# facebookresearch/SONAR

Hardware: NVIDIA B200
Metric: sentences/sec->1024-d (higher is better)
Workload: dtype bf16

## Files before the change

include/sonar_b200.h:

```cpp
#ifndef SONAR_B200_H_
#define SONAR_B200_H_

#include <stddef.h>
#include <stdint.h>

#ifdef __cplusplus
extern "C" {
#endif

#define SB_OK 0
#define SB_ERR_INVALID (-1)
#define SB_ERR_CUDA (-2)
#define SB_ERR_DRIVER (-3)
#define SB_ERR_INPUT (-4)

#define SB_POOL_MAX 1
#define SB_POOL_MEAN 2
#define SB_POOL_LAST 3

#define SB_EPI_BIAS 0
#define SB_EPI_BIAS_RELU 1
#define SB_EPI_BIAS_RESIDUAL 2
#define SB_EPI_BIAS_SILU 5

typedef struct SbEncoder SbEncoder;

typedef struct SbEncoderConfig {
  int32_t model_dim;
  int32_t num_layers;
  int32_t num_heads;
  int32_t ffn_inner_dim;
  int64_t vocab_size;
  int32_t pos_rows;
  int32_t pooling;
  float ln_eps;
  float embed_scale;
  int32_t cta_group;
  int32_t num_sms;
  int32_t ln_fold;
  int32_t epi_groups;
} SbEncoderConfig;

typedef struct SbLayerWeights {
  const void* wqkv;
  const float* bqkv;
  const void* wo;
  const float* bo;
  const void* w1;
  const float* b1;
  const void* w2;
  const float* b2;
  const float* ln1_g;
  const float* ln1_b;
  const float* ln2_g;
  const float* ln2_b;
} SbLayerWeights;

typedef struct SbEncoderWeights {
  const void* embed;
  const float* pos_table;
  const float* final_ln_g;
  const float* final_ln_b;
  const SbLayerWeights* layers;
} SbEncoderWeights;

const char* sb_last_error(void);
int sb_version(void);

int sb_encoder_create(const SbEncoderConfig* cfg, const SbEncoderWeights* w, SbEncoder** out);
void sb_encoder_destroy(SbEncoder* enc);

int sb_encoder_workspace_bytes(const SbEncoder* enc, int32_t max_batch, int64_t max_tokens, size_t* bytes);

int sb_encoder_forward(SbEncoder* enc, const int64_t* ids, int64_t ids_row_stride, const int32_t* seq_lens_host,
                       int32_t batch, int32_t seq_len, float* out, float* encoded, void* workspace,
                       size_t workspace_bytes, void* stream);

int sb_encoder_forward_host(SbEncoder* enc, const int64_t* ids_host, const int32_t* seq_lens_host, int32_t batch,
                            int32_t seq_len, float* out_host, int64_t* ids_staging, float* out_staging,
                            void* workspace, size_t workspace_bytes, void* stream);

int sb_encoder_profile_ffn1(SbEncoder* enc, void* start_event, void* stop_event);

int sb_encoder_check_inputs(SbEncoder* enc, void* workspace, void* stream);


int sb_fold_layernorm(const void* W, const float* bias, const float* gamma, const float* beta, int32_t N, int32_t K,
                      void* Wf, float* colsum, float* bias_f, void* stream);
int sb_gemm_ln_consumer(const void* A, int64_t lda, const void* Wf, int64_t ldw, void* C, int64_t ldc, const float* bias_f,
                        const float* colsum, const float* stats, float eps, int32_t M, int32_t N, int32_t K, int32_t relu,
                        void* stream);
int sb_gemm_residual_stats(const void* A, int64_t lda, const void* W, int64_t ldw, float* x, int64_t ldx, const float* bias,
                           void* h_out, int64_t ldh, float* stats_out, int32_t M, int32_t N, int32_t K, void* stream);

int sb_gemm_residual_splitk(const void* A, int64_t lda, const void* W, int64_t ldw, float* x, int64_t ldx, const float* bias,
                            int32_t M, int32_t N, int32_t K, int32_t* counters, int64_t n_counters, void* stream);

int sb_gemm_bf16(const void* A, int64_t lda, const void* W, int64_t ldw, void* C, int64_t ldc, int32_t out_fp32,
                 const float* bias, const void* residual, int64_t ldr, int32_t M, int32_t N, int32_t K, int32_t epi,
                 int32_t cta_group, void* stream);

int sb_layernorm(const float* x, const float* gamma, const float* beta, float eps, void* y, int64_t T, int32_t D,
                 void* stream);

int sb_attention(const void* qkv, const int32_t* cu_seqlens, int32_t B, int32_t max_len, int32_t H,
                 int64_t total_tokens, int32_t impl, void* out, void* stream);

int sb_embed(const int64_t* ids, int64_t ids_row_stride, const int32_t* cu_seqlens, int32_t B, int32_t S,
             const void* embed, int64_t vocab, const float* pos_table, int32_t pos_rows, int32_t D, float scale,
             float* x, int32_t* err_flag, void* stream);

int sb_pool(const float* x, const int32_t* cu_seqlens, int32_t B, int32_t D, const float* gamma, const float* beta,
            float eps, int32_t apply_ln, int32_t pool_mode, float* out, float* encoded_padded, int32_t S_padded,
            void* stream);

typedef struct SbDecoder SbDecoder;

typedef struct SbDecoderConfig {
  int32_t model_dim;
  int32_t num_layers;
  int32_t num_heads;
  int32_t ffn_inner_dim;
  int32_t input_dim;
  int64_t vocab_size;
  int32_t pos_rows;
  int32_t eos_idx;
  float ln_eps;
  float embed_scale;
} SbDecoderConfig;

typedef struct SbDecoderLayerWeights {
  const void* wqkv;
  const float* bqkv;
  const void* wo;
  const float* bo;
  const void* cross_wv;
  const float* cross_bv;
  const void* cross_wo;
  const float* cross_bo;
  const void* w1;
  const float* b1;
  const void* w2;
  const float* b2;
  const float* ln1_g;
  const float* ln1_b;
  const float* ln3_g;
  const float* ln3_b;
} SbDecoderLayerWeights;

typedef struct SbDecoderWeights {
  const void* embed;
  const float* pos_table;
  const float* final_ln_g;
  const float* final_ln_b;
  const SbDecoderLayerWeights* layers;
} SbDecoderWeights;

int sb_decoder_create(const SbDecoderConfig* cfg, const SbDecoderWeights* w, SbDecoder** out);
void sb_decoder_destroy(SbDecoder* dec);
int sb_decoder_workspace_bytes(const SbDecoder* dec, int32_t num_sentences, int32_t beam, int32_t max_len, size_t* bytes);
int sb_decoder_begin(SbDecoder* dec, const float* embeddings, int32_t num_sentences, int32_t beam, int32_t max_len,
                     void* workspace, size_t workspace_bytes, void* stream);
int sb_decoder_step(SbDecoder* dec, const int64_t* tokens, const int32_t* table, int32_t t, int32_t num_sentences,
                    int32_t beam, int32_t max_len, float* out_lprob, int32_t* out_tok, float* out_eos_lprob,
                    const int64_t* probe_tokens, float* out_probe_lprob, void* workspace, size_t workspace_bytes,
                    void* stream);
int sb_decoder_check_inputs(SbDecoder* dec, void* workspace, void* stream);

size_t sb_fbank_tables_bytes(void);
int sb_fbank_build_tables(void* host_buf);
int sb_fbank(const float* waves, const int64_t* wave_offsets, const int32_t* frame_offsets, int32_t B,
             int32_t total_frames, const void* tables, float* raw_out, float* out, int32_t padded_frames, void* stream);

typedef struct SbSpeechEncoder SbSpeechEncoder;

typedef struct SbSpeechConfig {
  int32_t model_dim;
  int32_t num_layers;
  int32_t num_heads;
  int32_t ffn_inner_dim;
  int32_t conv_kernel;
  int32_t pooler_layers;
  int32_t pooler_ffn_inner_dim;
  float ln_eps;
  int32_t attn_impl;
} SbSpeechConfig;

typedef struct SbConformerLayerWeights {
  const float* ffn1_ln_g; const float* ffn1_ln_b;
  const void* ffn1_w1; const float* ffn1_b1; const void* ffn1_w2 ; const float* ffn1_b2 ;
  const float* attn_ln_g; const float* attn_ln_b;
  const void* wqkv; const float* bqkv; const void* wo; const float* bo;
  const void* wr;
  const float* u_bias;
  const float* v_bias;
  const float* conv_ln_g; const float* conv_ln_b;
  const void* pw1;
  const float* dw;
  const float* bn_scale;
  const float* bn_shift;
  const void* pw2;
  const float* ffn2_ln_g; const float* ffn2_ln_b;
  const void* ffn2_w1; const float* ffn2_b1; const void* ffn2_w2 ; const float* ffn2_b2 ;
  const float* ln_g; const float* ln_b;
} SbConformerLayerWeights;

typedef struct SbPoolerLayerWeights {
  const void* sa_wv; const float* sa_bv; const void* sa_wo; const float* sa_bo;
  const float* sa_ln_g; const float* sa_ln_b;
  const void* ca_wq; const float* ca_bq;
  const void* ca_wkv ; const float* ca_bkv;
  const void* ca_wo; const float* ca_bo;
  const float* ca_ln_g; const float* ca_ln_b;
  const void* w1; const float* b1; const void* w2; const float* b2;
  const float* ffn_ln_g; const float* ffn_ln_b;
} SbPoolerLayerWeights;

typedef struct SbSpeechWeights {
  const float* front_ln_g;
  const float* front_ln_b;
  const void* front_w;
  const float* front_b;
  const float* final_ln_g;
  const float* final_ln_b;
  const float* pooler_q0;
  const void* proj_w;
  const float* zeros;
  const SbConformerLayerWeights* layers;
  const SbPoolerLayerWeights* pooler;
} SbSpeechWeights;

int sb_speech_encoder_create(const SbSpeechConfig* cfg, const SbSpeechWeights* w, SbSpeechEncoder** out);
void sb_speech_encoder_destroy(SbSpeechEncoder* enc);
int sb_speech_encoder_workspace_bytes(const SbSpeechEncoder* enc, int32_t batch, int64_t total_positions,
                                      int32_t max_positions, size_t* bytes);
int sb_speech_encoder_forward(SbSpeechEncoder* enc, const float* fbank, int32_t padded_frames, const int32_t* cu_dev,
                              const int32_t* lens_host, int32_t batch, const void* relpos_table, int32_t relpos_rows,
                              float* out, float* encoded_packed, void* workspace, size_t workspace_bytes, void* stream);


int sb_xsim_workspace_bytes(int32_t n, int32_t m, int32_t d, size_t* bytes);

int sb_xsim_knn(const float* x, const float* y, int32_t n, int32_t m, int32_t d, int32_t k, double* out_val,
                int32_t* out_idx, void* workspace, size_t workspace_bytes, void* stream);

int sb_xsim_bidir_workspace_bytes(int32_t n, int32_t m, int32_t d, size_t* bytes);
int sb_xsim_knn_bidir(const float* x, const float* y, int32_t n, int32_t m, int32_t d, int32_t k, double* val_xy,
                      int32_t* idx_xy, double* val_yx, int32_t* idx_yx, int32_t* overflow_flag, void* workspace,
                      size_t workspace_bytes, void* stream);

int sb_xsim_margin_predict(const double* val_xy, const int32_t* idx_xy, const double* val_yx, int32_t n, int32_t m,
                           int32_t k, int32_t margin_mode, int32_t* pred, void* stream);

int sb_beam_step(const float* lp, const int32_t* tok, const float* eos_lp, int64_t* seqs, int32_t* table,
                 int64_t* tokens, float* cum, uint8_t* alive, uint8_t* done, float* fin_score, int64_t* fin_seq,
                 int64_t* fin_len, int64_t* fin_count, int32_t N, int32_t beam, int32_t Tmax, int32_t t, int32_t g,
                 int32_t eos_block, int32_t max_gen, int64_t vocab, int32_t eos, int32_t unk, int32_t pad,
                 float unk_penalty, float score_div, int32_t normalize, void* stream);

#ifdef __cplusplus
}
#endif
#endif
```

sonar_b200/_lib.py:

```python

from __future__ import annotations

import ctypes as C
from pathlib import Path
from typing import Optional

_LIB_PATH = Path(__file__).resolve().parent / "lib" / "libsonar_b200.so"
_lib: Optional[C.CDLL] = None

SB_POOL_MAX, SB_POOL_MEAN, SB_POOL_LAST = 1, 2, 3
SB_EPI_BIAS, SB_EPI_BIAS_RELU, SB_EPI_BIAS_RESIDUAL = 0, 1, 2
SB_ERR_INVALID, SB_ERR_CUDA, SB_ERR_DRIVER, SB_ERR_INPUT = -1, -2, -3, -4


class SbEncoderConfig(C.Structure):
    _fields_ = [
        ("model_dim", C.c_int32), ("num_layers", C.c_int32), ("num_heads", C.c_int32),
        ("ffn_inner_dim", C.c_int32), ("vocab_size", C.c_int64), ("pos_rows", C.c_int32),
        ("pooling", C.c_int32), ("ln_eps", C.c_float), ("embed_scale", C.c_float),
        ("cta_group", C.c_int32), ("num_sms", C.c_int32), ("ln_fold", C.c_int32), ("epi_groups", C.c_int32),
    ]


class SbLayerWeights(C.Structure):
    _fields_ = [(n, C.c_void_p) for n in (
        "wqkv", "bqkv", "wo", "bo", "w1", "b1", "w2", "b2", "ln1_g", "ln1_b", "ln2_g", "ln2_b")]


class SbEncoderWeights(C.Structure):
    _fields_ = [("embed", C.c_void_p), ("pos_table", C.c_void_p), ("final_ln_g", C.c_void_p),
                ("final_ln_b", C.c_void_p), ("layers", C.POINTER(SbLayerWeights))]


class SbDecoderConfig(C.Structure):
    _fields_ = [
        ("model_dim", C.c_int32), ("num_layers", C.c_int32), ("num_heads", C.c_int32),
        ("ffn_inner_dim", C.c_int32), ("input_dim", C.c_int32), ("vocab_size", C.c_int64),
        ("pos_rows", C.c_int32), ("eos_idx", C.c_int32), ("ln_eps", C.c_float), ("embed_scale", C.c_float),
    ]


class SbDecoderLayerWeights(C.Structure):
    _fields_ = [(n, C.c_void_p) for n in (
        "wqkv", "bqkv", "wo", "bo", "cross_wv", "cross_bv", "cross_wo", "cross_bo", "w1", "b1", "w2", "b2",
        "ln1_g", "ln1_b", "ln3_g", "ln3_b")]


class SbDecoderWeights(C.Structure):
    _fields_ = [("embed", C.c_void_p), ("pos_table", C.c_void_p), ("final_ln_g", C.c_void_p),
                ("final_ln_b", C.c_void_p), ("layers", C.POINTER(SbDecoderLayerWeights))]


class SbSpeechConfig(C.Structure):
    _fields_ = [("model_dim", C.c_int32), ("num_layers", C.c_int32), ("num_heads", C.c_int32),
                ("ffn_inner_dim", C.c_int32), ("conv_kernel", C.c_int32), ("pooler_layers", C.c_int32),
                ("pooler_ffn_inner_dim", C.c_int32), ("ln_eps", C.c_float), ("attn_impl", C.c_int32)]


CONFORMER_FIELDS = ("ffn1_ln_g", "ffn1_ln_b", "ffn1_w1", "ffn1_b1", "ffn1_w2", "ffn1_b2", "attn_ln_g", "attn_ln_b",
                    "wqkv", "bqkv", "wo", "bo", "wr", "u_bias", "v_bias", "conv_ln_g", "conv_ln_b", "pw1", "dw",
                    "bn_scale", "bn_shift", "pw2", "ffn2_ln_g", "ffn2_ln_b", "ffn2_w1", "ffn2_b1", "ffn2_w2", "ffn2_b2",
                    "ln_g", "ln_b")
POOLER_FIELDS = ("sa_wv", "sa_bv", "sa_wo", "sa_bo", "sa_ln_g", "sa_ln_b", "ca_wq", "ca_bq", "ca_wkv", "ca_bkv",
                 "ca_wo", "ca_bo", "ca_ln_g", "ca_ln_b", "w1", "b1", "w2", "b2", "ffn_ln_g", "ffn_ln_b")


class SbConformerLayerWeights(C.Structure):
    _fields_ = [(n, C.c_void_p) for n in CONFORMER_FIELDS]


class SbPoolerLayerWeights(C.Structure):
    _fields_ = [(n, C.c_void_p) for n in POOLER_FIELDS]


class SbSpeechWeights(C.Structure):
    _fields_ = [(n, C.c_void_p) for n in ("front_ln_g", "front_ln_b", "front_w", "front_b", "final_ln_g", "final_ln_b",
                                          "pooler_q0", "proj_w", "zeros")] + \
               [("layers", C.POINTER(SbConformerLayerWeights)), ("pooler", C.POINTER(SbPoolerLayerWeights))]


_SIGNATURES = {
    "sb_last_error": (C.c_char_p, []),
    "sb_version": (C.c_int, []),
    "sb_encoder_create": (C.c_int, [C.POINTER(SbEncoderConfig), C.POINTER(SbEncoderWeights),
                                    C.POINTER(C.c_void_p)]),
    "sb_encoder_destroy": (None, [C.c_void_p]),
    "sb_encoder_workspace_bytes": (C.c_int, [C.c_void_p, C.c_int32, C.c_int64, C.POINTER(C.c_size_t)]),
    "sb_encoder_forward": (C.c_int, [C.c_void_p, C.c_void_p, C.c_int64, C.c_void_p, C.c_int32, C.c_int32,
                                     C.c_void_p, C.c_void_p, C.c_void_p, C.c_size_t, C.c_void_p]),
    "sb_encoder_forward_host": (C.c_int, [C.c_void_p, C.c_void_p, C.c_void_p, C.c_int32, C.c_int32,
                                          C.c_void_p, C.c_void_p, C.c_void_p, C.c_void_p, C.c_size_t,
                                          C.c_void_p]),
    "sb_encoder_profile_ffn1": (C.c_int, [C.c_void_p, C.c_void_p, C.c_void_p]),
    "sb_encoder_check_inputs": (C.c_int, [C.c_void_p, C.c_void_p, C.c_void_p]),
    "sb_gemm_bf16": (C.c_int, [C.c_void_p, C.c_int64, C.c_void_p, C.c_int64, C.c_void_p, C.c_int64,
                               C.c_int32, C.c_void_p, C.c_void_p, C.c_int64, C.c_int32, C.c_int32,
                               C.c_int32, C.c_int32, C.c_int32, C.c_void_p]),
    "sb_layernorm": (C.c_int, [C.c_void_p, C.c_void_p, C.c_void_p, C.c_float, C.c_void_p, C.c_int64,
                               C.c_int32, C.c_void_p]),
    "sb_attention": (C.c_int, [C.c_void_p, C.c_void_p, C.c_int32, C.c_int32, C.c_int32, C.c_int64, C.c_int32,
                               C.c_void_p, C.c_void_p]),
    "sb_embed": (C.c_int, [C.c_void_p, C.c_int64, C.c_void_p, C.c_int32, C.c_int32, C.c_void_p, C.c_int64,
                           C.c_void_p, C.c_int32, C.c_int32, C.c_float, C.c_void_p, C.c_void_p, C.c_void_p]),
    "sb_pool": (C.c_int, [C.c_void_p, C.c_void_p, C.c_int32, C.c_int32, C.c_void_p, C.c_void_p, C.c_float,
                          C.c_int32, C.c_int32, C.c_void_p, C.c_void_p, C.c_int32, C.c_void_p]),
    "sb_decoder_create": (C.c_int, [C.POINTER(SbDecoderConfig), C.POINTER(SbDecoderWeights), C.POINTER(C.c_void_p)]),
    "sb_decoder_destroy": (None, [C.c_void_p]),
    "sb_decoder_workspace_bytes": (C.c_int, [C.c_void_p, C.c_int32, C.c_int32, C.c_int32, C.POINTER(C.c_size_t)]),
    "sb_decoder_begin": (C.c_int, [C.c_void_p, C.c_void_p, C.c_int32, C.c_int32, C.c_int32, C.c_void_p, C.c_size_t,
                                   C.c_void_p]),
    "sb_decoder_step": (C.c_int, [C.c_void_p, C.c_void_p, C.c_void_p, C.c_int32, C.c_int32, C.c_int32, C.c_int32,
                                  C.c_void_p, C.c_void_p, C.c_void_p, C.c_void_p, C.c_void_p, C.c_void_p, C.c_size_t,
                                  C.c_void_p]),
    "sb_decoder_check_inputs": (C.c_int, [C.c_void_p, C.c_void_p, C.c_void_p]),
    "sb_fbank_tables_bytes": (C.c_size_t, []),
    "sb_fbank_build_tables": (C.c_int, [C.c_void_p]),
    "sb_fbank": (C.c_int, [C.c_void_p, C.c_void_p, C.c_void_p, C.c_int32, C.c_int32, C.c_void_p, C.c_void_p,
                           C.c_void_p, C.c_int32, C.c_void_p]),
    "sb_speech_encoder_create": (C.c_int, [C.POINTER(SbSpeechConfig), C.POINTER(SbSpeechWeights), C.POINTER(C.c_void_p)]),
    "sb_speech_encoder_destroy": (None, [C.c_void_p]),
    "sb_speech_encoder_workspace_bytes": (C.c_int, [C.c_void_p, C.c_int32, C.c_int64, C.c_int32, C.POINTER(C.c_size_t)]),
    "sb_speech_encoder_forward": (C.c_int, [C.c_void_p, C.c_void_p, C.c_int32, C.c_void_p, C.c_void_p, C.c_int32,
                                            C.c_void_p, C.c_int32, C.c_void_p, C.c_void_p, C.c_void_p, C.c_size_t,
                                            C.c_void_p]),
    "sb_xsim_workspace_bytes": (C.c_int, [C.c_int32, C.c_int32, C.c_int32, C.POINTER(C.c_size_t)]),
    "sb_xsim_knn": (C.c_int, [C.c_void_p, C.c_void_p, C.c_int32, C.c_int32, C.c_int32, C.c_int32, C.c_void_p,
                              C.c_void_p, C.c_void_p, C.c_size_t, C.c_void_p]),
    "sb_xsim_margin_predict": (C.c_int, [C.c_void_p, C.c_void_p, C.c_void_p, C.c_int32, C.c_int32, C.c_int32,
                                         C.c_int32, C.c_void_p, C.c_void_p]),
    "sb_fold_layernorm": (C.c_int, [C.c_void_p] * 4 + [C.c_int32, C.c_int32] + [C.c_void_p] * 4),
    "sb_gemm_ln_consumer": (C.c_int, [C.c_void_p, C.c_int64, C.c_void_p, C.c_int64, C.c_void_p, C.c_int64, C.c_void_p,
                                      C.c_void_p, C.c_void_p, C.c_float, C.c_int32, C.c_int32, C.c_int32, C.c_int32,
                                      C.c_void_p]),
    "sb_gemm_residual_stats": (C.c_int, [C.c_void_p, C.c_int64, C.c_void_p, C.c_int64, C.c_void_p, C.c_int64, C.c_void_p,
                                         C.c_void_p, C.c_int64, C.c_void_p, C.c_int32, C.c_int32, C.c_int32, C.c_void_p]),
    "sb_gemm_residual_splitk": (C.c_int, [C.c_void_p, C.c_int64, C.c_void_p, C.c_int64, C.c_void_p, C.c_int64, C.c_void_p,
                                          C.c_int32, C.c_int32, C.c_int32, C.c_void_p, C.c_int64, C.c_void_p]),
    "sb_xsim_bidir_workspace_bytes": (C.c_int, [C.c_int32, C.c_int32, C.c_int32, C.POINTER(C.c_size_t)]),
    "sb_xsim_knn_bidir": (C.c_int, [C.c_void_p, C.c_void_p, C.c_int32, C.c_int32, C.c_int32, C.c_int32, C.c_void_p, C.c_void_p,
                                    C.c_void_p, C.c_void_p, C.c_void_p, C.c_void_p, C.c_size_t, C.c_void_p]),
    "sb_beam_step": (C.c_int, [C.c_void_p] * 13 + [C.c_int32] * 7 + [C.c_int64] + [C.c_int32] * 3 +
                     [C.c_float, C.c_float, C.c_int32, C.c_void_p]),
}


def lib_path() -> Path:
    return _LIB_PATH


def load() -> C.CDLL:
    global _lib
    if _lib is not None:
        return _lib
    if not _LIB_PATH.exists():
        raise RuntimeError(
            f"sonar_b200: native library {_LIB_PATH} is missing -- run `python -m sonar_b200.build` "
            "(or `__graft_entry__.build()`); there is no CPU/PyTorch fallback path.")
    lib = C.CDLL(str(_LIB_PATH))
    for name, (restype, argtypes) in _SIGNATURES.items():
        fn = getattr(lib, name)
        fn.restype = restype
        fn.argtypes = argtypes
    _lib = lib
    return lib


def last_error() -> str:
    msg = load().sb_last_error()
    return msg.decode("utf-8", "replace") if msg else ""


def check(rc: int, what: str) -> None:
    if rc == 0:
        return
    msg = f"{what}: {last_error()} (code {rc})"
    if rc in (SB_ERR_INVALID, SB_ERR_INPUT):
        raise ValueError(msg)
    raise RuntimeError(msg)
```

sonar_b200/csrc/common.cuh:

```cuda
#pragma once

#include <cuda.h>
#include <cuda_bf16.h>
#include <cuda_runtime.h>
#include <stdint.h>
#include <stdio.h>

namespace sb {

void set_last_error(const char* fmt, ...);

#define SB_CUDA_CHECK(expr)                                                              \
  do {                                                                                   \
    cudaError_t _e = (expr);                                                             \
    if (_e != cudaSuccess) {                                                             \
      ::sb::set_last_error("%s failed: %s (%s:%d)", #expr, cudaGetErrorString(_e),       \
                           __FILE__, __LINE__);                                          \
      return -2;                                                                         \
    }                                                                                    \
  } while (0)

__device__ __forceinline__ uint32_t smem_u32(const void* p) {
  return static_cast<uint32_t>(__cvta_generic_to_shared(p));
}

__device__ __forceinline__ uint32_t lane_id() {
  uint32_t l;
  asm volatile("mov.u32 %0, %%laneid;" : "=r"(l));
  return l;
}

__device__ __forceinline__ uint32_t cluster_ctarank() {
  uint32_t r;
  asm volatile("mov.u32 %0, %%cluster_ctarank;" : "=r"(r));
  return r;
}

__device__ __forceinline__ bool elect_one() {
  uint32_t pred = 0;
  asm volatile(
      "{\n\t"
      ".reg .pred p;\n\t"
      "elect.sync _|p, 0xffffffff;\n\t"
      "selp.u32 %0, 1, 0, p;\n\t"
      "}\n"
      : "=r"(pred));
  return pred != 0;
}

__device__ __forceinline__ void cluster_sync_all() {
  asm volatile("barrier.cluster.arrive.release.aligned;\n\t"
               "barrier.cluster.wait.acquire.aligned;\n" ::: "memory");
}

__device__ __forceinline__ void named_bar_sync(uint32_t id, uint32_t nthreads) {
  asm volatile("bar.sync %0, %1;" ::"r"(id), "r"(nthreads) : "memory");
}

__device__ __forceinline__ void mbar_init(uint64_t* bar, uint32_t count) {
  asm volatile("mbarrier.init.shared::cta.b64 [%0], %1;" ::"r"(smem_u32(bar)), "r"(count) : "memory");
}

__device__ __forceinline__ void fence_mbar_init() {
  asm volatile("fence.mbarrier_init.release.cluster;" ::: "memory");
}

__device__ __forceinline__ void mbar_arrive_expect_tx(uint64_t* bar, uint32_t bytes) {
  asm volatile("mbarrier.arrive.expect_tx.shared::cta.b64 _, [%0], %1;" ::"r"(smem_u32(bar)), "r"(bytes)
               : "memory");
}

__device__ __forceinline__ void mbar_arrive(uint64_t* bar) {
  asm volatile("mbarrier.arrive.shared::cta.b64 _, [%0];" ::"r"(smem_u32(bar)) : "memory");
}

__device__ __forceinline__ void mbar_arrive_cluster(uint64_t* bar, uint32_t cta) {
  asm volatile(
      "{\n\t"
      ".reg .b32 ra;\n\t"
      "mapa.shared::cluster.u32 ra, %0, %1;\n\t"
      "mbarrier.arrive.release.cluster.shared::cluster.b64 _, [ra];\n\t"
      "}\n" ::"r"(smem_u32(bar)),
      "r"(cta)
      : "memory");
}

__device__ __forceinline__ bool mbar_try_wait(uint64_t* bar, uint32_t parity) {
  uint32_t ok;
  asm volatile(
      "{\n\t"
      ".reg .pred p;\n\t"
      "mbarrier.try_wait.parity.shared::cta.b64 p, [%1], %2;\n\t"
      "selp.u32 %0, 1, 0, p;\n\t"
      "}\n"
      : "=r"(ok)
      : "r"(smem_u32(bar)), "r"(parity)
      : "memory");
  return ok != 0;
}

__device__ __forceinline__ bool mbar_test_wait(uint64_t* bar, uint32_t parity) {
  uint32_t ok;
  asm volatile(
      "{\n\t"
      ".reg .pred p;\n\t"
      "mbarrier.test_wait.parity.shared::cta.b64 p, [%1], %2;\n\t"
      "selp.u32 %0, 1, 0, p;\n\t"
      "}\n"
      : "=r"(ok)
      : "r"(smem_u32(bar)), "r"(parity)
      : "memory");
  return ok != 0;
}

#ifndef SB_MBAR_TIMEOUT_CYCLES
#define SB_MBAR_TIMEOUT_CYCLES (4000000000ll)
#endif
__device__ __forceinline__ void mbar_wait(uint64_t* bar, uint32_t parity) {
  if (mbar_try_wait(bar, parity)) return;
  const long long t0 = clock64();
  while (!mbar_try_wait(bar, parity)) {
    if (clock64() - t0 > SB_MBAR_TIMEOUT_CYCLES) {
      printf("sonar_b200: mbarrier timeout block=(%d,%d) thread=%d bar=%u parity=%u\n", blockIdx.x,
             blockIdx.y, threadIdx.x, smem_u32(bar), parity);
      __trap();
    }
  }
}

__device__ __forceinline__ void tma_prefetch_desc(const CUtensorMap* m) {
  asm volatile("prefetch.tensormap [%0];" ::"l"(reinterpret_cast<uint64_t>(m)) : "memory");
}

__device__ __forceinline__ void tma_load_2d(void* smem_dst, const CUtensorMap* m, uint64_t* bar, int c0,
                                            int c1) {
  asm volatile(
      "cp.async.bulk.tensor.2d.shared::cluster.global.mbarrier::complete_tx::bytes [%0], [%1, {%3, %4}], [%2];" ::"r"(
          smem_u32(smem_dst)),
      "l"(reinterpret_cast<uint64_t>(m)), "r"(smem_u32(bar)), "r"(c0), "r"(c1)
      : "memory");
}

__device__ __forceinline__ void tma_load_2d_cta2(void* smem_dst, const CUtensorMap* m, uint64_t* bar, int c0,
                                                 int c1) {
  uint32_t bar_addr = smem_u32(bar) & 0xFEFFFFFFu;
  asm volatile(
      "cp.async.bulk.tensor.2d.cta_group::2.shared::cluster.global.mbarrier::complete_tx::bytes [%0], [%1, {%3, "
      "%4}], [%2];" ::"r"(smem_u32(smem_dst)),
      "l"(reinterpret_cast<uint64_t>(m)), "r"(bar_addr), "r"(c0), "r"(c1)
      : "memory");
}

__device__ __forceinline__ void tma_store_2d(const CUtensorMap* m, const void* smem_src, int c0, int c1) {
  asm volatile("cp.async.bulk.tensor.2d.global.shared::cta.bulk_group [%0, {%2, %3}], [%1];" ::"l"(
                   reinterpret_cast<uint64_t>(m)),
               "r"(smem_u32(smem_src)), "r"(c0), "r"(c1)
               : "memory");
}

__device__ __forceinline__ void tma_reduce_add_2d(const CUtensorMap* m, const void* smem_src, int c0, int c1) {
  asm volatile("cp.reduce.async.bulk.tensor.2d.global.shared::cta.add.bulk_group [%0, {%2, %3}], [%1];" ::"l"(
                   reinterpret_cast<uint64_t>(m)),
               "r"(smem_u32(smem_src)), "r"(c0), "r"(c1)
               : "memory");
}

__device__ __forceinline__ void tma_store_commit() { asm volatile("cp.async.bulk.commit_group;" ::: "memory"); }

template <int N>
__device__ __forceinline__ void tma_store_wait_read() {
  asm volatile("cp.async.bulk.wait_group.read %0;" ::"n"(N) : "memory");
}

template <int N>
__device__ __forceinline__ void tma_store_wait_all() {
  asm volatile("cp.async.bulk.wait_group %0;" ::"n"(N) : "memory");
}

__device__ __forceinline__ void fence_proxy_async_all() { asm volatile("fence.proxy.async;" ::: "memory"); }
__device__ __forceinline__ int ld_acquire_gpu(const int* p) {
  int v;
  asm volatile("ld.acquire.gpu.global.s32 %0, [%1];" : "=r"(v) : "l"(p) : "memory");
  return v;
}
__device__ __forceinline__ void st_release_gpu(int* p, int v) {
  asm volatile("st.release.gpu.global.s32 [%0], %1;" ::"l"(p), "r"(v) : "memory");
}

__device__ __forceinline__ void fence_proxy_async_smem() {
  asm volatile("fence.proxy.async.shared::cta;" ::: "memory");
}

template <int kCtaGroup>
__device__ __forceinline__ void tmem_alloc(uint32_t* smem_dst, uint32_t ncols) {
  if constexpr (kCtaGroup == 1) {
    asm volatile("tcgen05.alloc.cta_group::1.sync.aligned.shared::cta.b32 [%0], %1;" ::"r"(smem_u32(smem_dst)),
                 "r"(ncols)
                 : "memory");
    asm volatile("tcgen05.relinquish_alloc_permit.cta_group::1.sync.aligned;" ::: "memory");
  } else {
    asm volatile("tcgen05.alloc.cta_group::2.sync.aligned.shared::cta.b32 [%0], %1;" ::"r"(smem_u32(smem_dst)),
                 "r"(ncols)
                 : "memory");
    asm volatile("tcgen05.relinquish_alloc_permit.cta_group::2.sync.aligned;" ::: "memory");
  }
}

template <int kCtaGroup>
__device__ __forceinline__ void tmem_dealloc(uint32_t taddr, uint32_t ncols) {
  if constexpr (kCtaGroup == 1) {
    asm volatile("tcgen05.dealloc.cta_group::1.sync.aligned.b32 %0, %1;" ::"r"(taddr), "r"(ncols) : "memory");
  } else {
    asm volatile("tcgen05.dealloc.cta_group::2.sync.aligned.b32 %0, %1;" ::"r"(taddr), "r"(ncols) : "memory");
  }
}

__device__ __forceinline__ void tc_fence_before() {
  asm volatile("tcgen05.fence::before_thread_sync;" ::: "memory");
}
__device__ __forceinline__ void tc_fence_after() {
  asm volatile("tcgen05.fence::after_thread_sync;" ::: "memory");
}

template <int kCtaGroup>
__device__ __forceinline__ void umma_bf16(uint32_t d_tmem, uint64_t a_desc, uint64_t b_desc, uint32_t idesc,
                                          uint32_t accumulate) {
  if constexpr (kCtaGroup == 1) {
    asm volatile(
        "{\n\t"
        ".reg .pred p;\n\t"
        "setp.ne.b32 p, %4, 0;\n\t"
        "tcgen05.mma.cta_group::1.kind::f16 [%0], %1, %2, %3, p;\n\t"
        "}\n" ::"r"(d_tmem),
        "l"(a_desc), "l"(b_desc), "r"(idesc), "r"(accumulate)
        : "memory");
  } else {
    asm volatile(
        "{\n\t"
        ".reg .pred p;\n\t"
        "setp.ne.b32 p, %4, 0;\n\t"
        "tcgen05.mma.cta_group::2.kind::f16 [%0], %1, %2, %3, p;\n\t"
        "}\n" ::"r"(d_tmem),
        "l"(a_desc), "l"(b_desc), "r"(idesc), "r"(accumulate)
        : "memory");
  }
}

template <int kCtaGroup>
__device__ __forceinline__ void umma_commit(uint64_t* bar, uint16_t cta_mask = 0x3) {
  if constexpr (kCtaGroup == 1) {
    asm volatile("tcgen05.commit.cta_group::1.mbarrier::arrive::one.shared::cluster.b64 [%0];" ::"r"(smem_u32(bar))
                 : "memory");
  } else {
    asm volatile(
        "tcgen05.commit.cta_group::2.mbarrier::arrive::one.shared::cluster.multicast::cluster.b64 [%0], %1;" ::"r"(
            smem_u32(bar)),
        "h"(cta_mask)
        : "memory");
  }
}

__device__ __forceinline__ void tmem_ld_32x32(uint32_t taddr, uint32_t (&v)[32]) {
  asm volatile(
      "tcgen05.ld.sync.aligned.32x32b.x32.b32 "
      "{%0, %1, %2, %3, %4, %5, %6, %7, %8, %9, %10, %11, %12, %13, %14, %15, "
      "%16, %17, %18, %19, %20, %21, %22, %23, %24, %25, %26, %27, %28, %29, %30, %31}, [%32];"
      : "=r"(v[0]), "=r"(v[1]), "=r"(v[2]), "=r"(v[3]), "=r"(v[4]), "=r"(v[5]), "=r"(v[6]), "=r"(v[7]),
        "=r"(v[8]), "=r"(v[9]), "=r"(v[10]), "=r"(v[11]), "=r"(v[12]), "=r"(v[13]), "=r"(v[14]), "=r"(v[15]),
        "=r"(v[16]), "=r"(v[17]), "=r"(v[18]), "=r"(v[19]), "=r"(v[20]), "=r"(v[21]), "=r"(v[22]), "=r"(v[23]),
        "=r"(v[24]), "=r"(v[25]), "=r"(v[26]), "=r"(v[27]), "=r"(v[28]), "=r"(v[29]), "=r"(v[30]), "=r"(v[31])
      : "r"(taddr)
      : "memory");
}

__device__ __forceinline__ void tmem_ld_wait() { asm volatile("tcgen05.wait::ld.sync.aligned;" ::: "memory"); }

__device__ __forceinline__ void tmem_st_32x16(uint32_t taddr, const uint32_t (&v)[16]) {
  asm volatile(
      "tcgen05.st.sync.aligned.32x32b.x16.b32 [%0], "
      "{%1, %2, %3, %4, %5, %6, %7, %8, %9, %10, %11, %12, %13, %14, %15, %16};" ::"r"(taddr),
      "r"(v[0]), "r"(v[1]), "r"(v[2]), "r"(v[3]), "r"(v[4]), "r"(v[5]), "r"(v[6]), "r"(v[7]), "r"(v[8]), "r"(v[9]),
      "r"(v[10]), "r"(v[11]), "r"(v[12]), "r"(v[13]), "r"(v[14]), "r"(v[15])
      : "memory");
}

__device__ __forceinline__ void tmem_st_wait() { asm volatile("tcgen05.wait::st.sync.aligned;" ::: "memory"); }

__device__ __forceinline__ void umma_bf16_ts(uint32_t d_tmem, uint32_t a_tmem, uint64_t b_desc, uint32_t idesc,
                                             uint32_t accumulate) {
  asm volatile(
      "{\n\t"
      ".reg .pred p;\n\t"
      "setp.ne.b32 p, %4, 0;\n\t"
      "tcgen05.mma.cta_group::1.kind::f16 [%0], [%1], %2, %3, p;\n\t"
      "}\n" ::"r"(d_tmem),
      "r"(a_tmem), "l"(b_desc), "r"(idesc), "r"(accumulate)
      : "memory");
}

__device__ __forceinline__ uint64_t umma_desc_kmajor_sw128(uint32_t smem_addr) {
  uint64_t lo = (smem_addr >> 4) & 0x3FFFu;
  uint64_t hi = (1024u >> 4)
                | (1u << 14)
                | (2u << 29);
  return lo | (hi << 32);
}

__host__ __device__ constexpr uint32_t umma_idesc_bf16_f32(uint32_t m, uint32_t n) {
  return (1u << 4)
         | (1u << 7)
         | (1u << 10)
         | ((n >> 3) << 17)
         | ((m >> 4) << 24);
}

__device__ __forceinline__ uint32_t pack_bf16x2(float lo, float hi) {
  __nv_bfloat162 v = __floats2bfloat162_rn(lo, hi);
  return *reinterpret_cast<uint32_t*>(&v);
}

__device__ __forceinline__ float warp_sum(float v) {
#pragma unroll
  for (int o = 16; o > 0; o >>= 1) v += __shfl_xor_sync(0xffffffffu, v, o);
  return v;
}
__device__ __forceinline__ float warp_max(float v) {
#pragma unroll
  for (int o = 16; o > 0; o >>= 1) v = fmaxf(v, __shfl_xor_sync(0xffffffffu, v, o));
  return v;
}

}

namespace sb {
static constexpr int kMaxVec = 8;

template <bool kL2 = false>
__device__ __forceinline__ void load_row(const float* row, int nvec, int lane, float4 (&v)[kMaxVec]) {
#pragma unroll
  for (int i = 0; i < kMaxVec; ++i)
    if (i < nvec) v[i] = kL2 ? __ldcg(reinterpret_cast<const float4*>(row + (i * 32 + lane) * 4))
                        : *reinterpret_cast<const float4*>(row + (i * 32 + lane) * 4);
}

__device__ __forceinline__ void normalize_row(float4 (&v)[kMaxVec], int nvec, int lane, int D,
                                              const float* __restrict__ gamma, const float* __restrict__ beta,
                                              float eps) {
  float s = 0.f;
#pragma unroll
  for (int i = 0; i < kMaxVec; ++i)
    if (i < nvec) s += (v[i].x + v[i].y) + (v[i].z + v[i].w);
  const float mean = warp_sum(s) / float(D);
  float q = 0.f;
#pragma unroll
  for (int i = 0; i < kMaxVec; ++i)
    if (i < nvec) {
      const float a = v[i].x - mean, b = v[i].y - mean, c = v[i].z - mean, d = v[i].w - mean;
      q += (a * a + b * b) + (c * c + d * d);
    }
  const float rstd = 1.0f / sqrtf(warp_sum(q) / float(D) + eps);
#pragma unroll
  for (int i = 0; i < kMaxVec; ++i)
    if (i < nvec) {
      const float4 g = __ldg(reinterpret_cast<const float4*>(gamma) + i * 32 + lane);
      const float4 bt = __ldg(reinterpret_cast<const float4*>(beta) + i * 32 + lane);
      v[i].x = (v[i].x - mean) * rstd * g.x + bt.x;
      v[i].y = (v[i].y - mean) * rstd * g.y + bt.y;
      v[i].z = (v[i].z - mean) * rstd * g.z + bt.z;
      v[i].w = (v[i].w - mean) * rstd * g.w + bt.w;
    }
}

}

__device__ __forceinline__ float tanh_approx(float x) {
  float y;
  asm("tanh.approx.f32 %0, %1;" : "=f"(y) : "f"(x));
  return y;
}
__device__ __forceinline__ float sigmoid_fast(float x) { return fmaf(0.5f, tanh_approx(0.5f * x), 0.5f); }
__device__ __forceinline__ float silu_fast(float x) {
  const float h = 0.5f * x;
  return fmaf(h, tanh_approx(h), h);
}
```

sonar_b200/csrc/encoder.cu:

```cuda

#include "../../include/sonar_b200.h"
#include <stdlib.h>

#include "common.cuh"
#include "sonar_b200_internal.h"

#include <cstdarg>
#include <cstdio>
#include <cstring>
#include <new>
#include <vector>

namespace sb {

static thread_local char g_err[512] = "";

void set_last_error(const char* fmt, ...) {
  va_list ap;
  va_start(ap, fmt);
  vsnprintf(g_err, sizeof(g_err), fmt, ap);
  va_end(ap);
}

static inline size_t align_up(size_t v, size_t a) { return (v + a - 1) / a * a; }

struct Workspace {
  int32_t* cu;
  float* ln_stats;
  float* x;
  __nv_bfloat16* h;
  __nv_bfloat16* qkv;
  __nv_bfloat16* f;
  size_t bytes;
};

}

using namespace sb;

struct FoldedLayer {
  __nv_bfloat16* wqkv = nullptr;
  __nv_bfloat16* w1 = nullptr;
  float* cqkv = nullptr;
  float* bqkv = nullptr;
  float* c1 = nullptr;
  float* b1 = nullptr;
};

struct SbEncoder {
  SbEncoderConfig cfg;
  std::vector<FoldedLayer> folded;
  void* fold_pool = nullptr;
  int32_t* err_flag = nullptr;
  const void* embed;
  const float* pos_table;
  const float* final_ln_g;
  const float* final_ln_b;
  std::vector<SbLayerWeights> layers;
  int num_sms;
  static constexpr int kSlots = 8;
  static constexpr int kSlotInts = 32768 + 8;
  int32_t* pinned = nullptr;
  cudaEvent_t ev[kSlots];
  bool ev_ok[kSlots];
  unsigned next_slot = 0;
  cudaEvent_t prof_start = nullptr, prof_stop = nullptr;
};

static Workspace carve(const SbEncoder* e, int32_t max_batch, int64_t max_tokens, void* base) {
  const size_t D = e->cfg.model_dim, F = e->cfg.ffn_inner_dim;
  const size_t T = (size_t)(max_tokens > 0 ? max_tokens : 1);
  uint8_t* p = reinterpret_cast<uint8_t*>(base);
  size_t off = 0;
  Workspace w;
  w.cu = reinterpret_cast<int32_t*>(p + off);
  off = align_up(off + sizeof(int32_t) * ((size_t)max_batch + 1), 1024);
  w.ln_stats = reinterpret_cast<float*>(p + off);
  off = align_up(off + T * (D / kLnPartCols) * 2 * sizeof(float), 1024);
  w.x = reinterpret_cast<float*>(p + off);
  off = align_up(off + T * D * 4, 1024);
  w.h = reinterpret_cast<__nv_bfloat16*>(p + off);
  off = align_up(off + T * D * 2, 1024);
  w.qkv = reinterpret_cast<__nv_bfloat16*>(p + off);
  off = align_up(off + T * 3 * D * 2, 1024);
  w.f = reinterpret_cast<__nv_bfloat16*>(p + off);
  off = align_up(off + T * F * 2, 1024);
  w.bytes = off;
  return w;
}

extern "C" {

const char* sb_last_error(void) { return g_err; }
int sb_version(void) { return 102; }

int sb_encoder_create(const SbEncoderConfig* cfg, const SbEncoderWeights* w, SbEncoder** out) {
  if (!cfg || !w || !out) { set_last_error("sb_encoder_create: null argument"); return SB_ERR_INVALID; }
  *out = nullptr;
  const int D = cfg->model_dim, H = cfg->num_heads, F = cfg->ffn_inner_dim;
  if (D <= 0 || D % 256 != 0 || D > 1024) {
    set_last_error("sb_encoder_create: model_dim must be a multiple of 256 and <= 1024 (got %d)", D);
    return SB_ERR_INVALID;
  }
  if (H <= 0 || D != H * 64) {
    set_last_error("sb_encoder_create: head_dim must be 64 (model_dim=%d, num_heads=%d)", D, H);
    return SB_ERR_INVALID;
  }
  if (F <= 0 || F % 256 != 0) { set_last_error("sb_encoder_create: ffn_inner_dim must be a multiple of 256"); return SB_ERR_INVALID; }
  if (cfg->ln_fold < 0 || cfg->ln_fold > 2) { set_last_error("sb_encoder_create: ln_fold must be 0, 1 or 2"); return SB_ERR_INVALID; }
  if (cfg->epi_groups < 0 || cfg->epi_groups > 2) { set_last_error("sb_encoder_create: epi_groups must be 0, 1 or 2"); return SB_ERR_INVALID; }
  if (cfg->epi_groups == 1 && (cfg->ln_fold != 0 || cfg->cta_group == 1)) {
    set_last_error("sb_encoder_create: epi_groups = 1 (the one-warpgroup epilogue kept for A/B runs) needs ln_fold = 0 and paired CTAs");
    return SB_ERR_INVALID;
  }
  if (cfg->num_layers < 0 || cfg->pos_rows <= 0 || cfg->vocab_size <= 0) {
    set_last_error("sb_encoder_create: bad num_layers / pos_rows / vocab_size");
    return SB_ERR_INVALID;
  }
  if (cfg->pooling != SB_POOL_MAX && cfg->pooling != SB_POOL_MEAN && cfg->pooling != SB_POOL_LAST) {
    set_last_error("sb_encoder_create: unsupported pooling %d", cfg->pooling);
    return SB_ERR_INVALID;
  }
  if (!w->embed || !w->pos_table || !w->final_ln_g || !w->final_ln_b || (cfg->num_layers > 0 && !w->layers)) {
    set_last_error("sb_encoder_create: missing weight pointer");
    return SB_ERR_INVALID;
  }
  int dev = 0, n_gpu = 0;
  if (cudaGetDeviceCount(&n_gpu) != cudaSuccess || n_gpu == 0) {
    set_last_error("sb_encoder_create: no CUDA device (this engine has no CPU path)");
    return SB_ERR_CUDA;
  }
  SB_CUDA_CHECK(cudaGetDevice(&dev));
  cudaDeviceProp prop;
  SB_CUDA_CHECK(cudaGetDeviceProperties(&prop, dev));
  if (prop.major != 10) {
    set_last_error("sb_encoder_create: sm_100a kernels need a Blackwell B200-class GPU (found sm_%d%d)", prop.major,
                   prop.minor);
    return SB_ERR_CUDA;
  }
  SbEncoder* e = new (std::nothrow) SbEncoder();
  if (!e) { set_last_error("out of host memory"); return SB_ERR_INVALID; }
  e->cfg = *cfg;
  e->embed = w->embed;
  e->pos_table = w->pos_table;
  e->final_ln_g = w->final_ln_g;
  e->final_ln_b = w->final_ln_b;
  e->layers.assign(w->layers, w->layers + cfg->num_layers);
  for (int i = 0; i < cfg->num_layers; ++i) {
    const SbLayerWeights& l = e->layers[i];
    if (!l.wqkv || !l.bqkv || !l.wo || !l.bo || !l.w1 || !l.b1 || !l.w2 || !l.b2 || !l.ln1_g || !l.ln1_b ||
        !l.ln2_g || !l.ln2_b) {
      set_last_error("sb_encoder_create: layer %d has a null weight pointer", i);
      delete e;
      return SB_ERR_INVALID;
    }
  }
  e->num_sms = cfg->num_sms > 0 ? cfg->num_sms : prop.multiProcessorCount;
  for (int i = 0; i < SbEncoder::kSlots; ++i) e->ev_ok[i] = false;
  if (cudaMallocHost(reinterpret_cast<void**>(&e->pinned), sizeof(int32_t) * SbEncoder::kSlots * SbEncoder::kSlotInts) !=
      cudaSuccess) {
    set_last_error("sb_encoder_create: cudaMallocHost failed");
    delete e;
    return SB_ERR_CUDA;
  }
  if (cudaMalloc(reinterpret_cast<void**>(&e->err_flag), 256) != cudaSuccess ||
      cudaMemset(e->err_flag, 0, 256) != cudaSuccess) {
    set_last_error("sb_encoder_create: cudaMalloc of the input-check flag failed");
    sb_encoder_destroy(e);
    return SB_ERR_CUDA;
  }
  if (cfg->ln_fold && cfg->num_layers > 0) {
    const size_t D_ = D, F_ = F;
    const size_t per_layer = align_up(3 * D_ * D_ * 2, 256) + align_up(F_ * D_ * 2, 256) + 2 * align_up(3 * D_ * 4, 256) +
                             2 * align_up(F_ * 4, 256);
    if (cudaMalloc(&e->fold_pool, per_layer * cfg->num_layers) != cudaSuccess) {
      set_last_error("sb_encoder_create: cudaMalloc of %zu bytes for the LayerNorm-folded weights failed",
                     per_layer * cfg->num_layers);
      sb_encoder_destroy(e);
      return SB_ERR_CUDA;
    }
    e->folded.resize(cfg->num_layers);
    uint8_t* p = reinterpret_cast<uint8_t*>(e->fold_pool);
    for (int i = 0; i < cfg->num_layers; ++i) {
      FoldedLayer& f = e->folded[i];
      const SbLayerWeights& l = e->layers[i];
      f.wqkv = reinterpret_cast<__nv_bfloat16*>(p); p += align_up(3 * D_ * D_ * 2, 256);
      f.w1 = reinterpret_cast<__nv_bfloat16*>(p); p += align_up(F_ * D_ * 2, 256);
      f.cqkv = reinterpret_cast<float*>(p); p += align_up(3 * D_ * 4, 256);
      f.bqkv = reinterpret_cast<float*>(p); p += align_up(3 * D_ * 4, 256);
      f.c1 = reinterpret_cast<float*>(p); p += align_up(F_ * 4, 256);
      f.b1 = reinterpret_cast<float*>(p); p += align_up(F_ * 4, 256);
      int rc = fold_layernorm_weights(reinterpret_cast<const __nv_bfloat16*>(l.wqkv), l.bqkv, l.ln1_g, l.ln1_b, 3 * D, D,
                                      f.wqkv, f.cqkv, f.bqkv, nullptr);
      if (!rc)
        rc = fold_layernorm_weights(reinterpret_cast<const __nv_bfloat16*>(l.w1), l.b1, l.ln2_g, l.ln2_b, F, D, f.w1, f.c1,
                                    f.b1, nullptr);
      if (rc) { sb_encoder_destroy(e); return rc; }
    }
    if (cudaDeviceSynchronize() != cudaSuccess) {
      set_last_error("sb_encoder_create: folding the LayerNorm weights failed: %s", cudaGetErrorString(cudaGetLastError()));
      sb_encoder_destroy(e);
      return SB_ERR_CUDA;
    }
  }
  for (int i = 0; i < SbEncoder::kSlots; ++i) {
    if (cudaEventCreateWithFlags(&e->ev[i], cudaEventDisableTiming) != cudaSuccess) {
      set_last_error("sb_encoder_create: cudaEventCreate failed");
      sb_encoder_destroy(e);
      return SB_ERR_CUDA;
    }
    e->ev_ok[i] = true;
  }
  *out = e;
  return SB_OK;
}

void sb_encoder_destroy(SbEncoder* e) {
  if (!e) return;
  for (int i = 0; i < SbEncoder::kSlots; ++i)
    if (e->ev_ok[i]) cudaEventDestroy(e->ev[i]);
  if (e->pinned) cudaFreeHost(e->pinned);
  if (e->fold_pool) cudaFree(e->fold_pool);
  if (e->err_flag) cudaFree(e->err_flag);
  delete e;
}

int sb_encoder_workspace_bytes(const SbEncoder* enc, int32_t max_batch, int64_t max_tokens, size_t* bytes) {
  if (!enc || !bytes || max_batch <= 0 || max_tokens <= 0) {
    set_last_error("sb_encoder_workspace_bytes: bad argument");
    return SB_ERR_INVALID;
  }
  *bytes = carve(enc, max_batch, max_tokens, nullptr).bytes + 1024;
  return SB_OK;
}

int sb_encoder_forward(SbEncoder* e, const int64_t* ids, int64_t ids_row_stride, const int32_t* seq_lens_host,
                       int32_t B, int32_t S, float* out, float* encoded, void* workspace, size_t workspace_bytes,
                       void* stream_v) {
  if (!e || !ids || !out || !workspace) { set_last_error("sb_encoder_forward: null argument"); return SB_ERR_INVALID; }
  if (B <= 0 || S <= 0) { set_last_error("sb_encoder_forward: empty batch (B=%d, S=%d)", B, S); return SB_ERR_INVALID; }
  if (S > e->cfg.pos_rows) {
    set_last_error("sb_encoder_forward: seq_len %d exceeds the encoder's max_seq_len %d", S, e->cfg.pos_rows);
    return SB_ERR_INVALID;
  }
  if (B + 1 > SbEncoder::kSlotInts) { set_last_error("sb_encoder_forward: batch too large (%d)", B); return SB_ERR_INVALID; }
  if (ids_row_stride < S) { set_last_error("sb_encoder_forward: ids_row_stride < seq_len"); return SB_ERR_INVALID; }
  cudaStream_t stream = reinterpret_cast<cudaStream_t>(stream_v);
  const int D = e->cfg.model_dim, F = e->cfg.ffn_inner_dim, H = e->cfg.num_heads;

  const unsigned slot = e->next_slot++ % SbEncoder::kSlots;
  SB_CUDA_CHECK(cudaEventSynchronize(e->ev[slot]));
  int32_t* cu_h = e->pinned + (size_t)slot * SbEncoder::kSlotInts;
  long long T = 0;
  int max_len = 0;
  cu_h[0] = 0;
  for (int b = 0; b < B; ++b) {
    const int len = seq_lens_host ? seq_lens_host[b] : S;
    if (len < 0 || len > S) { set_last_error("sb_encoder_forward: seq_lens[%d]=%d outside [0,%d]", b, len, S); return SB_ERR_INVALID; }
    T += len;
    if (len > max_len) max_len = len;
    if (T > 0x7fffffffll) { set_last_error("sb_encoder_forward: too many tokens"); return SB_ERR_INVALID; }
    cu_h[b + 1] = (int32_t)T;
  }
  uintptr_t base = (reinterpret_cast<uintptr_t>(workspace) + 1023) & ~uintptr_t(1023);
  Workspace w = carve(e, B, T, reinterpret_cast<void*>(base));
  if (base - reinterpret_cast<uintptr_t>(workspace) + w.bytes > workspace_bytes) {
    set_last_error("sb_encoder_forward: workspace too small (%zu bytes given, %zu needed for B=%d T=%lld)",
                   workspace_bytes, (size_t)(base - reinterpret_cast<uintptr_t>(workspace)) + w.bytes, B, T);
    return SB_ERR_INVALID;
  }
  SB_CUDA_CHECK(cudaMemcpyAsync(w.cu, cu_h, sizeof(int32_t) * (B + 1), cudaMemcpyHostToDevice, stream));
  SB_CUDA_CHECK(cudaEventRecord(e->ev[slot], stream));
  if (T == 0) {
    SB_CUDA_CHECK(cudaMemsetAsync(out, 0, sizeof(float) * (size_t)B * D, stream));
    return SB_OK;
  }

  const bool fold = e->cfg.ln_fold != 0 && e->cfg.num_layers > 0;
  const bool fold2 = fold && e->cfg.ln_fold == 1;
  __nv_bfloat16* hn = w.qkv;
  int rc;
  if ((rc = embed_tokens(ids, ids_row_stride, w.cu, B, S, reinterpret_cast<const __nv_bfloat16*>(e->embed),
                         e->cfg.vocab_size, e->pos_table, e->cfg.pos_rows, D, e->cfg.embed_scale, w.x, e->err_flag,
                         stream, 0, fold ? w.h : nullptr, fold ? w.ln_stats : nullptr)))
    return rc;

  GemmArgs g;
  g.cta_group = (e->cfg.cta_group == 1) ? 1 : 2;
  g.num_sms = e->num_sms;
  g.M = (int)T;
  g.epi_groups = (e->cfg.epi_groups == 1) ? 1 : 2;
  LnFold consume;
  consume.stats_in = w.ln_stats;
  consume.chunks = D / kLnPartCols;
  consume.eps = e->cfg.ln_eps;
  for (int li = 0; li < e->cfg.num_layers; ++li) {
    const SbLayerWeights& L = e->layers[li];
    if (!fold)
      if ((rc = layernorm_bf16(w.x, L.ln1_g, L.ln1_b, e->cfg.ln_eps, w.h, T, D, stream))) return rc;
    g.A = w.h; g.lda = D; g.ldw = D;
    g.C = w.qkv; g.ldc = 3 * D; g.out_fp32 = 0; g.residual = nullptr; g.ldr = 0;
    g.N = 3 * D; g.K = D; g.epi = EPI_BIAS;
    if (fold) {
      const FoldedLayer& f = e->folded[li];
      g.W = f.wqkv; g.bias = f.bqkv; g.lf = consume; g.lf.colsum = f.cqkv;
    } else {
      g.W = reinterpret_cast<const __nv_bfloat16*>(L.wqkv); g.bias = L.bqkv;
    }
    rc = gemm_bf16(g, stream);
    g.lf = LnFold();
    if (rc) return rc;
    if ((rc = attention_packed(w.qkv, w.cu, B, max_len, H, T, 0, e->num_sms, w.h, stream))) return rc;
    g.A = w.h; g.lda = D; g.W = reinterpret_cast<const __nv_bfloat16*>(L.wo); g.ldw = D;
    g.C = w.x; g.ldc = D; g.out_fp32 = 1; g.bias = L.bo; g.residual = w.x; g.ldr = D;
    g.N = D; g.K = D; g.epi = EPI_BIAS_RESIDUAL;
    if (fold2) {
      g.epi = EPI_BIAS_RESIDUAL_STATS;
      g.lf.h_out = hn; g.lf.ldh = D; g.lf.stats_out = w.ln_stats;
    }
    rc = gemm_bf16(g, stream);
    g.lf = LnFold();
    if (rc) return rc;
    if (!fold2)
      if ((rc = layernorm_bf16(w.x, L.ln2_g, L.ln2_b, e->cfg.ln_eps, w.h, T, D, stream))) return rc;
    g.A = fold2 ? hn : w.h; g.lda = D; g.ldw = D;
    g.C = w.f; g.ldc = F; g.out_fp32 = 0; g.residual = nullptr; g.ldr = 0;
    g.N = F; g.K = D; g.epi = EPI_BIAS_RELU;
    if (fold2) {
      const FoldedLayer& f = e->folded[li];
      g.W = f.w1; g.bias = f.b1; g.lf = consume; g.lf.colsum = f.c1;
    } else {
      g.W = reinterpret_cast<const __nv_bfloat16*>(L.w1); g.bias = L.b1;
    }
    const bool prof = e->prof_start && li == e->cfg.num_layers / 2;
    if (prof) SB_CUDA_CHECK(cudaEventRecord(e->prof_start, stream));
    rc = gemm_bf16(g, stream);
    g.lf = LnFold();
    if (rc) return rc;
    if (prof) SB_CUDA_CHECK(cudaEventRecord(e->prof_stop, stream));
    g.A = w.f; g.lda = F; g.W = reinterpret_cast<const __nv_bfloat16*>(L.w2); g.ldw = F;
    g.C = w.x; g.ldc = D; g.out_fp32 = 1; g.bias = L.b2; g.residual = w.x; g.ldr = D;
    g.N = D; g.K = F; g.epi = EPI_BIAS_RESIDUAL;
    if (fold && li + 1 < e->cfg.num_layers) {
      g.epi = EPI_BIAS_RESIDUAL_STATS;
      g.lf.h_out = w.h; g.lf.ldh = D; g.lf.stats_out = w.ln_stats;
    }
    rc = gemm_bf16(g, stream);
    g.lf = LnFold();
    if (rc) return rc;
  }
  return ln_pool(w.x, w.cu, B, D, e->final_ln_g, e->final_ln_b, e->cfg.ln_eps, 1, e->cfg.pooling, out, encoded, S,
                 stream);
}

int sb_encoder_forward_host(SbEncoder* e, const int64_t* ids_host, const int32_t* seq_lens_host, int32_t B,
                            int32_t S, float* out_host, int64_t* ids_staging, float* out_staging, void* workspace,
                            size_t workspace_bytes, void* stream_v) {
  if (!e || !ids_host || !out_host || !ids_staging || !out_staging) {
    set_last_error("sb_encoder_forward_host: null argument");
    return SB_ERR_INVALID;
  }
  if (B <= 0 || S <= 0) { set_last_error("sb_encoder_forward_host: empty batch"); return SB_ERR_INVALID; }
  cudaStream_t stream = reinterpret_cast<cudaStream_t>(stream_v);
  SB_CUDA_CHECK(cudaMemcpyAsync(ids_staging, ids_host, sizeof(int64_t) * (size_t)B * S, cudaMemcpyHostToDevice, stream));
  int rc = sb_encoder_forward(e, ids_staging, S, seq_lens_host, B, S, out_staging, nullptr, workspace, workspace_bytes,
                              stream_v);
  if (rc) return rc;
  SB_CUDA_CHECK(cudaMemcpyAsync(out_host, out_staging, sizeof(float) * (size_t)B * e->cfg.model_dim,
                                cudaMemcpyDeviceToHost, stream));
  SB_CUDA_CHECK(cudaStreamSynchronize(stream));
  return SB_OK;
}

int sb_encoder_profile_ffn1(SbEncoder* e, void* start_event, void* stop_event) {
  if (!e || (!start_event) != (!stop_event)) { set_last_error("sb_encoder_profile_ffn1: bad argument"); return SB_ERR_INVALID; }
  e->prof_start = reinterpret_cast<cudaEvent_t>(start_event);
  e->prof_stop = reinterpret_cast<cudaEvent_t>(stop_event);
  return SB_OK;
}

int sb_encoder_check_inputs(SbEncoder* e, void* workspace, void* stream_v) {
  (void)workspace;
  if (!e) { set_last_error("sb_encoder_check_inputs: null argument"); return SB_ERR_INVALID; }
  cudaStream_t stream = reinterpret_cast<cudaStream_t>(stream_v);
  int32_t flag = 0;
  SB_CUDA_CHECK(cudaMemcpyAsync(&flag, e->err_flag, sizeof(int32_t), cudaMemcpyDeviceToHost, stream));
  SB_CUDA_CHECK(cudaMemsetAsync(e->err_flag, 0, sizeof(int32_t), stream));
  SB_CUDA_CHECK(cudaStreamSynchronize(stream));
  if (flag != 0) {
    set_last_error("token id outside [0, vocab_size) in a batch passed to sb_encoder_forward since the last check");
    return SB_ERR_INPUT;
  }
  return SB_OK;
}

int sb_gemm_bf16(const void* A, int64_t lda, const void* W, int64_t ldw, void* C, int64_t ldc, int32_t out_fp32,
                 const float* bias, const void* residual, int64_t ldr, int32_t M, int32_t N, int32_t K, int32_t epi,
                 int32_t cta_group, void* stream) {
  if (!A || !W || !C) { set_last_error("sb_gemm_bf16: null pointer"); return SB_ERR_INVALID; }
  GemmArgs g;
  g.A = reinterpret_cast<const __nv_bfloat16*>(A); g.lda = lda;
  g.W = reinterpret_cast<const __nv_bfloat16*>(W); g.ldw = ldw;
  g.C = C; g.ldc = ldc; g.out_fp32 = out_fp32; g.bias = bias; g.residual = residual; g.ldr = ldr;
  g.M = M; g.N = N; g.K = K; g.epi = epi;
  g.cta_group = cta_group == 1 ? 1 : 2;
  g.allow_skinny = (cta_group == 0);
  int dev = 0, sms = 0;
  SB_CUDA_CHECK(cudaGetDevice(&dev));
  SB_CUDA_CHECK(cudaDeviceGetAttribute(&sms, cudaDevAttrMultiProcessorCount, dev));
  g.num_sms = sms;
  return gemm_bf16(g, reinterpret_cast<cudaStream_t>(stream));
}

int sb_fold_layernorm(const void* W, const float* bias, const float* gamma, const float* beta, int32_t N, int32_t K,
                      void* Wf, float* colsum, float* bias_f, void* stream) {
  if (!W || !bias || !gamma || !beta || !Wf || !colsum || !bias_f || N <= 0 || K <= 0) {
    set_last_error("sb_fold_layernorm: bad argument");
    return SB_ERR_INVALID;
  }
  return fold_layernorm_weights(reinterpret_cast<const __nv_bfloat16*>(W), bias, gamma, beta, N, K,
                                reinterpret_cast<__nv_bfloat16*>(Wf), colsum, bias_f, reinterpret_cast<cudaStream_t>(stream));
}

int sb_gemm_ln_consumer(const void* A, int64_t lda, const void* Wf, int64_t ldw, void* C, int64_t ldc, const float* bias_f,
                        const float* colsum, const float* stats, float eps, int32_t M, int32_t N, int32_t K, int32_t relu,
                        void* stream) {
  if (!A || !Wf || !C || !bias_f || !colsum || !stats) { set_last_error("sb_gemm_ln_consumer: null pointer"); return SB_ERR_INVALID; }
  GemmArgs g;
  g.A = reinterpret_cast<const __nv_bfloat16*>(A); g.lda = lda;
  g.W = reinterpret_cast<const __nv_bfloat16*>(Wf); g.ldw = ldw;
  g.C = C; g.ldc = ldc; g.out_fp32 = 0; g.bias = bias_f; g.residual = nullptr; g.ldr = 0;
  g.M = M; g.N = N; g.K = K; g.epi = relu ? EPI_BIAS_RELU : EPI_BIAS;
  g.cta_group = 2;
  g.lf.stats_in = stats; g.lf.colsum = colsum; g.lf.chunks = K / kLnPartCols; g.lf.eps = eps;
  int dev = 0, sms = 0;
  SB_CUDA_CHECK(cudaGetDevice(&dev));
  SB_CUDA_CHECK(cudaDeviceGetAttribute(&sms, cudaDevAttrMultiProcessorCount, dev));
  g.num_sms = sms;
  return gemm_bf16(g, reinterpret_cast<cudaStream_t>(stream));
}

int sb_gemm_residual_stats(const void* A, int64_t lda, const void* W, int64_t ldw, float* x, int64_t ldx, const float* bias,
                           void* h_out, int64_t ldh, float* stats_out, int32_t M, int32_t N, int32_t K, void* stream) {
  if (!A || !W || !x || !bias || !h_out || !stats_out) { set_last_error("sb_gemm_residual_stats: null pointer"); return SB_ERR_INVALID; }
  GemmArgs g;
  g.A = reinterpret_cast<const __nv_bfloat16*>(A); g.lda = lda;
  g.W = reinterpret_cast<const __nv_bfloat16*>(W); g.ldw = ldw;
  g.C = x; g.ldc = ldx; g.out_fp32 = 1; g.bias = bias; g.residual = x; g.ldr = ldx;
  g.M = M; g.N = N; g.K = K; g.epi = EPI_BIAS_RESIDUAL_STATS;
  g.cta_group = 2;
  g.lf.h_out = reinterpret_cast<__nv_bfloat16*>(h_out); g.lf.ldh = ldh; g.lf.stats_out = stats_out;
  int dev = 0, sms = 0;
  SB_CUDA_CHECK(cudaGetDevice(&dev));
  SB_CUDA_CHECK(cudaDeviceGetAttribute(&sms, cudaDevAttrMultiProcessorCount, dev));
  g.num_sms = sms;
  return gemm_bf16(g, reinterpret_cast<cudaStream_t>(stream));
}

int sb_gemm_residual_splitk(const void* A, int64_t lda, const void* W, int64_t ldw, float* x, int64_t ldx, const float* bias,
                            int32_t M, int32_t N, int32_t K, int32_t* counters, int64_t n_counters, void* stream) {
  if (!A || !W || !x || !bias || !counters) { set_last_error("sb_gemm_residual_splitk: null pointer"); return SB_ERR_INVALID; }
  GemmArgs g;
  g.A = reinterpret_cast<const __nv_bfloat16*>(A); g.lda = lda;
  g.W = reinterpret_cast<const __nv_bfloat16*>(W); g.ldw = ldw;
  g.C = x; g.ldc = ldx; g.out_fp32 = 1; g.bias = bias; g.residual = x; g.ldr = ldx;
  g.M = M; g.N = N; g.K = K; g.epi = EPI_BIAS_RESIDUAL;
  g.cta_group = 2;
  g.splitk_flags = counters;
  g.splitk_flags_len = n_counters;
  int dev = 0, sms = 0;
  SB_CUDA_CHECK(cudaGetDevice(&dev));
  SB_CUDA_CHECK(cudaDeviceGetAttribute(&sms, cudaDevAttrMultiProcessorCount, dev));
  g.num_sms = sms;
  return gemm_bf16(g, reinterpret_cast<cudaStream_t>(stream));
}

int sb_layernorm(const float* x, const float* gamma, const float* beta, float eps, void* y, int64_t T, int32_t D,
                 void* stream) {
  if (!x || !gamma || !beta || !y) { set_last_error("sb_layernorm: null pointer"); return SB_ERR_INVALID; }
  return layernorm_bf16(x, gamma, beta, eps, reinterpret_cast<__nv_bfloat16*>(y), T, D,
                        reinterpret_cast<cudaStream_t>(stream));
}

int sb_attention(const void* qkv, const int32_t* cu_seqlens, int32_t B, int32_t max_len, int32_t H,
                 int64_t total_tokens, int32_t impl, void* out, void* stream) {
  if (!qkv || !cu_seqlens || !out) { set_last_error("sb_attention: null pointer"); return SB_ERR_INVALID; }
  int dev = 0, sms = 0;
  SB_CUDA_CHECK(cudaGetDevice(&dev));
  SB_CUDA_CHECK(cudaDeviceGetAttribute(&sms, cudaDevAttrMultiProcessorCount, dev));
  return attention_packed(reinterpret_cast<const __nv_bfloat16*>(qkv), cu_seqlens, B, max_len, H, total_tokens, impl,
                          sms, reinterpret_cast<__nv_bfloat16*>(out), reinterpret_cast<cudaStream_t>(stream));
}

int sb_embed(const int64_t* ids, int64_t ids_row_stride, const int32_t* cu_seqlens, int32_t B, int32_t S,
             const void* embed, int64_t vocab, const float* pos_table, int32_t pos_rows, int32_t D, float scale,
             float* x, int32_t* err_flag, void* stream) {
  if (!ids || !cu_seqlens || !embed || !pos_table || !x || !err_flag) {
    set_last_error("sb_embed: null pointer");
    return SB_ERR_INVALID;
  }
  return embed_tokens(ids, ids_row_stride, cu_seqlens, B, S, reinterpret_cast<const __nv_bfloat16*>(embed), vocab,
                      pos_table, pos_rows, D, scale, x, err_flag, reinterpret_cast<cudaStream_t>(stream));
}

int sb_pool(const float* x, const int32_t* cu_seqlens, int32_t B, int32_t D, const float* gamma, const float* beta,
            float eps, int32_t apply_ln, int32_t pool_mode, float* out, float* encoded_padded, int32_t S_padded,
            void* stream) {
  if (!x || !cu_seqlens || !out) { set_last_error("sb_pool: null pointer"); return SB_ERR_INVALID; }
  return ln_pool(x, cu_seqlens, B, D, gamma, beta, eps, apply_ln, pool_mode, out, encoded_padded, S_padded,
                 reinterpret_cast<cudaStream_t>(stream));
}

}
```

sonar_b200/csrc/gemm_tcgen05.cu:

```cuda

#include "common.cuh"
#include "sonar_b200_internal.h"

#include <math_constants.h>

namespace sb {

template <int kCtaGroup, int kEpiGroups = 2>
struct GemmCfg {
  static constexpr int BLOCK_M = 128;
  static constexpr int BLOCK_N = 256;
  static constexpr int BLOCK_K = 64;
  static constexpr int LOAD_N = BLOCK_N / kCtaGroup;
  static constexpr int A_BYTES = BLOCK_M * BLOCK_K * 2;
  static constexpr int B_BYTES = LOAD_N * BLOCK_K * 2;
  static constexpr int STAGES = (kCtaGroup == 2) ? (kEpiGroups == 2 ? 5 : 6) : (kEpiGroups == 2 ? 3 : 4);
  static constexpr int CD_STAGE_BYTES = 128 * 128;
  static constexpr int EPI_GROUPS = kEpiGroups;
  static constexpr int CD_STAGES = 2;
  static constexpr int BAR_BYTES = 256;
  static constexpr int SMEM_BYTES =
      STAGES * (A_BYTES + B_BYTES) + EPI_GROUPS * CD_STAGES * CD_STAGE_BYTES + BAR_BYTES + 1024 ;
  static constexpr int TMEM_COLS = 512;
  static constexpr int THREADS = 128 + 128 * EPI_GROUPS;
};

template <bool kSweep>
struct TileSched {
  int num_m_tiles, num_n_tiles, cluster_id, num_clusters, n_chunks, tiles_per_chunk;
  int k_splits = 1;
  int i = 0, j = 0;
  __device__ __forceinline__ bool next(int& m_blk, int& n_blk, int& chunk, bool& first, bool& last) {
    if constexpr (!kSweep) {
      const int item = cluster_id + i * num_clusters;
      ++i;
      const int tiles = num_m_tiles * num_n_tiles;
      if (item >= tiles * k_splits) return false;
      const int tile = (k_splits == 1) ? item : item % tiles;
      chunk = (k_splits == 1) ? 0 : item / tiles;
      m_blk = tile / num_n_tiles;
      n_blk = tile % num_n_tiles;
      first = last = true;
      return true;
    } else {
      for (;;) {
        const int item = cluster_id + i * num_clusters;
        if (item >= num_m_tiles * n_chunks) return false;
        m_blk = item / n_chunks;
        chunk = item % n_chunks;
        const int n_begin = chunk * tiles_per_chunk;
        const int cnt = min(tiles_per_chunk, num_n_tiles - n_begin);
        if (j < cnt) {
          n_blk = n_begin + j;
          first = (j == 0);
          last = (j == cnt - 1);
          ++j;
          return true;
        }
        j = 0;
        ++i;
      }
    }
  }
};

template <int KC>
__device__ __forceinline__ void topk_insert(float (&tv)[KC], int (&ti)[KC], float v, int idx) {
  float cv = v;
  int ci = idx;
#pragma unroll
  for (int p = 0; p < KC; ++p) {
    const bool gt = cv > tv[p];
    const float ov = tv[p];
    const int oi = ti[p];
    tv[p] = gt ? cv : ov;
    ti[p] = gt ? ci : oi;
    cv = gt ? ov : cv;
    ci = gt ? oi : ci;
  }
}

template <int kCtaGroup, int kEpi, typename OutT, int kEpiGroups>
__global__ void __launch_bounds__(GemmCfg<kCtaGroup, kEpiGroups>::THREADS, 1)
gemm_bf16_tcgen05_kernel(const __grid_constant__ CUtensorMap tm_a, const __grid_constant__ CUtensorMap tm_b,
                         const __grid_constant__ CUtensorMap tm_c, const float* __restrict__ bias,
                         const OutT* residual, long long ldr, int M, int N, int K, float* __restrict__ cand_val,
                         int* __restrict__ cand_idx, float* __restrict__ lse_part, int n_chunks, const LnFold lf,
                         const ColFilter cf, int k_splits, int* __restrict__ splitk_flags) {
  constexpr bool kSweep = (kEpi == EPI_TOPK);
  using Cfg = GemmCfg<kCtaGroup, kEpiGroups>;
  extern __shared__ uint8_t smem_raw[];
  uint8_t* smem = reinterpret_cast<uint8_t*>((reinterpret_cast<uintptr_t>(smem_raw) + 1023) & ~uintptr_t(1023));
  uint8_t* smem_a = smem;
  uint8_t* smem_b = smem_a + Cfg::STAGES * Cfg::A_BYTES;
  uint8_t* smem_cd = smem_b + Cfg::STAGES * Cfg::B_BYTES;
  uint64_t* full_bar = reinterpret_cast<uint64_t*>(smem_cd + Cfg::EPI_GROUPS * Cfg::CD_STAGES * Cfg::CD_STAGE_BYTES);
  uint64_t* empty_bar = full_bar + Cfg::STAGES;
  uint64_t* tmem_full_bar = empty_bar + Cfg::STAGES;
  uint64_t* tmem_empty_bar = tmem_full_bar + 2;
  uint32_t* tmem_ptr_smem = reinterpret_cast<uint32_t*>(tmem_empty_bar + 2);

  const int warp_idx = threadIdx.x >> 5;
  const int lane = threadIdx.x & 31;
  const uint32_t cta_rank = (kCtaGroup == 2) ? cluster_ctarank() : 0u;
  const bool is_leader = (cta_rank == 0);

  if (kCtaGroup == 2) cluster_sync_all();

  if (warp_idx == 0 && lane == 0) {
    tma_prefetch_desc(&tm_a);
    tma_prefetch_desc(&tm_b);
    tma_prefetch_desc(&tm_c);
  }
  if (warp_idx == 1 && lane == 0) {
    for (int i = 0; i < Cfg::STAGES; ++i) {
      mbar_init(&full_bar[i], 1);
      mbar_init(&empty_bar[i], 1);
    }
    for (int i = 0; i < 2; ++i) {
      mbar_init(&tmem_full_bar[i], 1);
      mbar_init(&tmem_empty_bar[i], 4 * Cfg::EPI_GROUPS * kCtaGroup);
    }
    fence_mbar_init();
  }
  if (warp_idx == 2) tmem_alloc<kCtaGroup>(tmem_ptr_smem, Cfg::TMEM_COLS);
  tc_fence_before();
  if (kCtaGroup == 2) cluster_sync_all(); else __syncthreads();
  tc_fence_after();
  const uint32_t tmem_base = *tmem_ptr_smem;

  const int tile_m = Cfg::BLOCK_M * kCtaGroup;
  const int num_m_tiles = (M + tile_m - 1) / tile_m;
  const int num_n_tiles = (N + Cfg::BLOCK_N - 1) / Cfg::BLOCK_N;
  const int num_kb = K / Cfg::BLOCK_K;
  const int cluster_id = blockIdx.x / kCtaGroup;
  const int num_clusters = gridDim.x / kCtaGroup;
  TileSched<kSweep> sched{num_m_tiles, num_n_tiles, cluster_id, num_clusters, n_chunks,
                          (num_n_tiles + n_chunks - 1) / n_chunks, (kEpi == EPI_BIAS_ACCUM) ? k_splits : 1};
  auto kb_begin = [&](int split) { return (kEpi == EPI_BIAS_ACCUM && k_splits > 1) ? split * num_kb / k_splits : 0; };
  auto kb_end = [&](int split) { return (kEpi == EPI_BIAS_ACCUM && k_splits > 1) ? (split + 1) * num_kb / k_splits : num_kb; };
  int m_blk, n_blk, chunk;
  bool first_in_item, last_in_item;

  if (warp_idx == 0) {
    if (lane == 0) {
      int stage = 0;
      uint32_t phase = 0;
      while (sched.next(m_blk, n_blk, chunk, first_in_item, last_in_item)) {
        const int m0 = m_blk * tile_m + int(cta_rank) * Cfg::BLOCK_M;
        const int n0 = n_blk * Cfg::BLOCK_N + int(cta_rank) * Cfg::LOAD_N;
        const int kb1 = kb_end(chunk);
        for (int kb = kb_begin(chunk); kb < kb1; ++kb) {
          mbar_wait(&empty_bar[stage], phase ^ 1);
          if (is_leader) mbar_arrive_expect_tx(&full_bar[stage], (Cfg::A_BYTES + Cfg::B_BYTES) * kCtaGroup);
          if (kCtaGroup == 2) {
            tma_load_2d_cta2(smem_a + stage * Cfg::A_BYTES, &tm_a, &full_bar[stage], kb * Cfg::BLOCK_K, m0);
            tma_load_2d_cta2(smem_b + stage * Cfg::B_BYTES, &tm_b, &full_bar[stage], kb * Cfg::BLOCK_K, n0);
          } else {
            tma_load_2d(smem_a + stage * Cfg::A_BYTES, &tm_a, &full_bar[stage], kb * Cfg::BLOCK_K, m0);
            tma_load_2d(smem_b + stage * Cfg::B_BYTES, &tm_b, &full_bar[stage], kb * Cfg::BLOCK_K, n0);
          }
          if (++stage == Cfg::STAGES) { stage = 0; phase ^= 1; }
        }
      }
    }
    __syncwarp();
  } else if (warp_idx == 1) {
    if (is_leader) {
      constexpr uint32_t idesc = umma_idesc_bf16_f32(Cfg::BLOCK_M * kCtaGroup, Cfg::BLOCK_N);
      constexpr uint32_t desc_hi = (1024u >> 4) | (1u << 14) | (2u << 29);
      const uint32_t a_lo0 = (smem_u32(smem_a) >> 4) & 0x3FFFu;
      const uint32_t b_lo0 = (smem_u32(smem_b) >> 4) & 0x3FFFu;
      int stage = 0;
      uint32_t phase = 0;
      for (uint32_t iter = 0; sched.next(m_blk, n_blk, chunk, first_in_item, last_in_item); ++iter) {
        const uint32_t acc = iter & 1, acc_phase = (iter >> 1) & 1;
        mbar_wait(&tmem_empty_bar[acc], acc_phase ^ 1);
        tc_fence_after();
        const uint32_t d_tmem = tmem_base + acc * Cfg::BLOCK_N;
        const int kb0 = kb_begin(chunk), kb1 = kb_end(chunk);
        for (int kb = kb0; kb < kb1; ++kb) {
          mbar_wait(&full_bar[stage], phase);
          tc_fence_after();
          if (elect_one()) {
            const uint32_t a_lo = a_lo0 + uint32_t(stage) * (Cfg::A_BYTES >> 4);
            const uint32_t b_lo = b_lo0 + uint32_t(stage) * (Cfg::B_BYTES >> 4);
#pragma unroll
            for (int k = 0; k < Cfg::BLOCK_K / 16; ++k) {
              const uint64_t a_desc = (uint64_t(desc_hi) << 32) | uint64_t(a_lo + 2 * k);
              const uint64_t b_desc = (uint64_t(desc_hi) << 32) | uint64_t(b_lo + 2 * k);
              umma_bf16<kCtaGroup>(d_tmem, a_desc, b_desc, idesc, ((kb - kb0) | k) != 0 ? 1u : 0u);
            }
            umma_commit<kCtaGroup>(&empty_bar[stage]);
            if (kb == kb1 - 1) umma_commit<kCtaGroup>(&tmem_full_bar[acc]);
          }
          __syncwarp();
          if (++stage == Cfg::STAGES) { stage = 0; phase ^= 1; }
        }
      }
    }
  } else if (warp_idx >= 4) {
    const int wg = (warp_idx - 4) >> 2;
    const int ew = warp_idx & 3;
    const int row_in_tile = ew * 32 + lane;
    constexpr int CHUNK_COLS = 128 / int(sizeof(OutT));
    constexpr int NUM_CHUNKS = Cfg::BLOCK_N / CHUNK_COLS;
    constexpr int SUBS = CHUNK_COLS / 32;
    static_assert(NUM_CHUNKS % Cfg::EPI_GROUPS == 0, "column chunks must split evenly over the epilogue warpgroups");
    uint8_t* smem_cd_wg = smem_cd + wg * Cfg::CD_STAGES * Cfg::CD_STAGE_BYTES;
    const uint32_t bar_id = 1 + wg;
    int cd_stage = 0;
    constexpr int KC = kTopkCandidates;
    [[maybe_unused]] float tv[KC];
    [[maybe_unused]] int ti[KC];
    [[maybe_unused]] float run_max = -CUDART_INF_F, run_sum = 0.f;
    [[maybe_unused]] int q_n = 0;
    [[maybe_unused]] bool fold_in = false;
    [[maybe_unused]] float2 part_next[8];
    [[maybe_unused]] TileSched<kSweep> sched_ahead = sched;
    [[maybe_unused]] auto fetch_parts = [&]() {
      int mb, nb, ch;
      bool f0, f1;
      if (!sched_ahead.next(mb, nb, ch, f0, f1)) return;
      const int r = mb * tile_m + int(cta_rank) * Cfg::BLOCK_M + row_in_tile;
      if (r < M) {
        const float2* sp = reinterpret_cast<const float2*>(lf.stats_in) + (long long)r * lf.chunks;
#pragma unroll
        for (int i = 0; i < 8; ++i)
          if (i < lf.chunks) part_next[i] = sp[i];
      }
    };
    if constexpr (kEpi == EPI_BIAS || kEpi == EPI_BIAS_RELU) {
      fold_in = lf.stats_in != nullptr;
      if (fold_in) fetch_parts();
    }
    for (uint32_t iter = 0; sched.next(m_blk, n_blk, chunk, first_in_item, last_in_item); ++iter) {
      const int m0 = m_blk * tile_m + int(cta_rank) * Cfg::BLOCK_M;
      const int n0 = n_blk * Cfg::BLOCK_N;
      const uint32_t acc = iter & 1, acc_phase = (iter >> 1) & 1;
      const int grow = m0 + row_in_tile;
      [[maybe_unused]] float ln_mean = 0.f, ln_rstd = 1.f;
      if constexpr (kEpi == EPI_BIAS || kEpi == EPI_BIAS_RELU) {
        if (fold_in) {
          if (grow < M) {
            float msum = 0.f;
#pragma unroll
            for (int i = 0; i < 8; ++i)
              if (i < lf.chunks) msum += part_next[i].x;
            ln_mean = msum / float(lf.chunks);
            float m2 = 0.f;
#pragma unroll
            for (int i = 0; i < 8; ++i)
              if (i < lf.chunks) { const float dm = part_next[i].x - ln_mean; m2 += part_next[i].y + float(kLnPartCols) * dm * dm; }
            ln_rstd = 1.0f / sqrtf(m2 / float(kLnPartCols * lf.chunks) + lf.eps);
          }
          fetch_parts();
        }
      }
      [[maybe_unused]] float4 rnext[8];
      [[maybe_unused]] float st_n = 0.f, st_mean = 0.f, st_m2 = 0.f;
      if constexpr (kEpi == EPI_BIAS_RESIDUAL_STATS) {
#pragma unroll
        for (int q = 0; q < 8; ++q) rnext[q] = make_float4(0.f, 0.f, 0.f, 0.f);
        if (grow < M) {
          const float4* rp = reinterpret_cast<const float4*>(reinterpret_cast<const float*>(residual) + (long long)grow * ldr +
                                                             n0 + wg * CHUNK_COLS);
#pragma unroll
          for (int q = 0; q < 8; ++q) rnext[q] = rp[q];
        }
      }
      mbar_wait(&tmem_full_bar[acc], acc_phase);
      tc_fence_after();
      if constexpr (kEpi == EPI_TOPK) {
        if (first_in_item) {
#pragma unroll
          for (int p = 0; p < KC; ++p) { tv[p] = -CUDART_INF_F; ti[p] = -1; }
          run_max = -CUDART_INF_F;
          run_sum = 0.f;
        }
        const bool cf_on = cf.thr != nullptr && grow < M;
        constexpr int kQ = 16;
        uint2* queue = reinterpret_cast<uint2*>(smem_cd_wg) + row_in_tile;
        auto drain = [&]() {
          const int rounds = __reduce_max_sync(0xffffffffu, q_n);
          for (int r = 0; r < rounds; ++r) {
            if (r < q_n) {
              const uint2 e = queue[r * 128];
              const float x = __uint_as_float(e.x);
              if (x > tv[KC - 1]) topk_insert<KC>(tv, ti, x, int(e.y));
            }
          }
          q_n = 0;
        };
#pragma unroll 1
        for (int c = wg; c < Cfg::BLOCK_N / 32; c += Cfg::EPI_GROUPS) {
          uint32_t v[32];
          tmem_ld_32x32(tmem_base + (uint32_t(ew * 32) << 16) + acc * Cfg::BLOCK_N + c * 32, v);
          tmem_ld_wait();
          const int gcol = n0 + c * 32;
          if (gcol + 32 > N) {
#pragma unroll
            for (int j = 0; j < 32; ++j)
              if (gcol + j >= N) v[j] = __float_as_uint(-CUDART_INF_F);
          }
          float gm[4];
#pragma unroll
          for (int g8 = 0; g8 < 4; ++g8) {
            float mx = __uint_as_float(v[g8 * 8]);
#pragma unroll
            for (int j = 1; j < 8; ++j) mx = fmaxf(mx, __uint_as_float(v[g8 * 8 + j]));
            gm[g8] = mx;
          }
          if (lse_part != nullptr) {
            const float cm = fmaxf(fmaxf(gm[0], gm[1]), fmaxf(gm[2], gm[3]));
            if (cm > run_max) {
              run_sum *= __expf(run_max - cm);
              run_max = cm;
            }
            if (run_max > -CUDART_INF_F) {
              float cs = 0.f;
#pragma unroll
              for (int j = 0; j < 32; ++j) cs += __expf(__uint_as_float(v[j]) - run_max);
              run_sum += cs;
            }
          }
          const float thr = tv[KC - 1];
          float t8[4] = {CUDART_INF_F, CUDART_INF_F, CUDART_INF_F, CUDART_INF_F};
          if (cf_on) {
            const float4 t = __ldg(reinterpret_cast<const float4*>(cf.thr8 + (gcol >> 3)));
            t8[0] = t.x; t8[1] = t.y; t8[2] = t.z; t8[3] = t.w;
          }
#pragma unroll
          for (int g8 = 0; g8 < 4; ++g8) {
            if (gm[g8] > t8[g8]) {
              const float4 t0 = *reinterpret_cast<const float4*>(cf.thr + gcol + g8 * 8);
              const float4 t1 = *reinterpret_cast<const float4*>(cf.thr + gcol + g8 * 8 + 4);
              const float th[8] = {t0.x, t0.y, t0.z, t0.w, t1.x, t1.y, t1.z, t1.w};
#pragma unroll
              for (int j = 0; j < 8; ++j) {
                const float x = __uint_as_float(v[g8 * 8 + j]);
                if (x > th[j]) {
                  const int col = gcol + g8 * 8 + j;
                  const int slot = atomicAdd(cf.cnt + col, 1);
                  if (slot < cf.cap) cf.buf[(long long)col * cf.cap + slot] = make_uint2(__float_as_uint(x), uint32_t(grow));
                  else cf.thr[col] = CUDART_INF_F;
                }
              }
            }
            if (gm[g8] > thr) {
#pragma unroll
              for (int j = 0; j < 8; ++j) {
                const float x = __uint_as_float(v[g8 * 8 + j]);
                if (x > thr) {
                  queue[q_n * 128] = make_uint2(__float_as_uint(x), uint32_t(gcol + g8 * 8 + j));
                  ++q_n;
                }
              }
            }
            if (__any_sync(0xffffffffu, q_n > kQ - 8)) drain();
          }
        }
        if (last_in_item) drain();
        tc_fence_before();
        __syncwarp();
        if (lane == 0) {
          if (kCtaGroup == 2) mbar_arrive_cluster(&tmem_empty_bar[acc], 0);
          else mbar_arrive(&tmem_empty_bar[acc]);
        }
        if (last_in_item && grow < M) {
          const long long slot = ((long long)grow * n_chunks + chunk) * Cfg::EPI_GROUPS + wg;
#pragma unroll
          for (int p = 0; p < KC; ++p) {
            cand_val[slot * KC + p] = tv[p];
            cand_idx[slot * KC + p] = ti[p];
          }
          if (lse_part != nullptr) {
            lse_part[slot * 2] = run_max;
            lse_part[slot * 2 + 1] = run_sum;
          }
        }
        continue;
      }
#pragma unroll 1
      for (int c = wg; c < NUM_CHUNKS; c += Cfg::EPI_GROUPS) {
        if (ew == 0 && lane == 0) tma_store_wait_read<Cfg::CD_STAGES - 1>();
        named_bar_sync(bar_id, 128);
        uint8_t* cd_row = smem_cd_wg + cd_stage * Cfg::CD_STAGE_BYTES + row_in_tile * 128;
#pragma unroll
        for (int s = 0; s < SUBS; ++s) {
          uint32_t v[32];
          const int col_in_tile = c * CHUNK_COLS + s * 32;
          tmem_ld_32x32(tmem_base + (uint32_t(ew * 32) << 16) + acc * Cfg::BLOCK_N + col_in_tile, v);
          tmem_ld_wait();
          const int gcol = n0 + col_in_tile;
          float f[32];
          if (fold_in) {
#pragma unroll
            for (int j = 0; j < 32; j += 4) {
              const float4 b4 = __ldg(reinterpret_cast<const float4*>(bias + gcol + j));
              const float4 c4 = __ldg(reinterpret_cast<const float4*>(lf.colsum + gcol + j));
              f[j + 0] = fmaf(ln_rstd, fmaf(-ln_mean, c4.x, __uint_as_float(v[j + 0])), b4.x);
              f[j + 1] = fmaf(ln_rstd, fmaf(-ln_mean, c4.y, __uint_as_float(v[j + 1])), b4.y);
              f[j + 2] = fmaf(ln_rstd, fmaf(-ln_mean, c4.z, __uint_as_float(v[j + 2])), b4.z);
              f[j + 3] = fmaf(ln_rstd, fmaf(-ln_mean, c4.w, __uint_as_float(v[j + 3])), b4.w);
            }
          } else {
            const bool with_bias = !(kEpi == EPI_BIAS_ACCUM && chunk > 0);
#pragma unroll
            for (int j = 0; j < 32; j += 4) {
              const float4 b4 = with_bias ? __ldg(reinterpret_cast<const float4*>(bias + gcol + j)) : make_float4(0.f, 0.f, 0.f, 0.f);
              f[j + 0] = __uint_as_float(v[j + 0]) + b4.x;
              f[j + 1] = __uint_as_float(v[j + 1]) + b4.y;
              f[j + 2] = __uint_as_float(v[j + 2]) + b4.z;
              f[j + 3] = __uint_as_float(v[j + 3]) + b4.w;
            }
          }
          if constexpr (kEpi == EPI_BIAS_RESIDUAL_STATS) {
            float4 rcur[8];
#pragma unroll
            for (int q = 0; q < 8; ++q) rcur[q] = rnext[q];
            if (c + Cfg::EPI_GROUPS < NUM_CHUNKS && grow < M) {
              const float4* rp = reinterpret_cast<const float4*>(reinterpret_cast<const float*>(residual) +
                                                                 (long long)grow * ldr + gcol + Cfg::EPI_GROUPS * CHUNK_COLS);
#pragma unroll
              for (int q = 0; q < 8; ++q) rnext[q] = rp[q];
            }
#pragma unroll
            for (int q = 0; q < 8; ++q) {
              f[4 * q + 0] += rcur[q].x; f[4 * q + 1] += rcur[q].y; f[4 * q + 2] += rcur[q].z; f[4 * q + 3] += rcur[q].w;
            }
            float cs = 0.f;
#pragma unroll
            for (int j = 0; j < 32; ++j) cs += f[j];
            const float cm = cs * (1.0f / 32.0f);
            float cq = 0.f;
#pragma unroll
            for (int j = 0; j < 32; ++j) { const float dv = f[j] - cm; cq = fmaf(dv, dv, cq); }
            const float n_new = st_n + 32.f;
            const float dlt = cm - st_mean;
            st_mean = fmaf(dlt, 32.f / n_new, st_mean);
            st_m2 += cq + dlt * dlt * (st_n * 32.f / n_new);
            st_n = n_new;
            if (grow < M) {
              uint4* hp = reinterpret_cast<uint4*>(lf.h_out + (long long)grow * lf.ldh + gcol);
#pragma unroll
              for (int q = 0; q < 4; ++q)
                hp[q] = make_uint4(pack_bf16x2(f[8 * q], f[8 * q + 1]), pack_bf16x2(f[8 * q + 2], f[8 * q + 3]),
                                   pack_bf16x2(f[8 * q + 4], f[8 * q + 5]), pack_bf16x2(f[8 * q + 6], f[8 * q + 7]));
              if (c + Cfg::EPI_GROUPS >= NUM_CHUNKS)
                reinterpret_cast<float2*>(lf.stats_out)[((long long)grow * num_n_tiles + n_blk) * Cfg::EPI_GROUPS + wg] =
                    make_float2(st_mean, st_m2);
            }
          }
          if constexpr (kEpi == EPI_BIAS_RELU) {
#pragma unroll
            for (int j = 0; j < 32; ++j) f[j] = fmaxf(f[j], 0.0f);
          }
          if constexpr (kEpi == EPI_BIAS_SILU) {
#pragma unroll
            for (int j = 0; j < 32; ++j) f[j] = silu_fast(f[j]);
          }
          if constexpr (kEpi == EPI_BIAS_RESIDUAL) {
            if (grow < M) {
              const OutT* rp = residual + (long long)grow * ldr + gcol;
              if constexpr (sizeof(OutT) == 4) {
#pragma unroll
                for (int j = 0; j < 32; j += 4) {
                  const float4 r4 = *reinterpret_cast<const float4*>(reinterpret_cast<const float*>(rp) + j);
                  f[j + 0] += r4.x; f[j + 1] += r4.y; f[j + 2] += r4.z; f[j + 3] += r4.w;
                }
              } else {
#pragma unroll
                for (int j = 0; j < 32; j += 8) {
                  const uint4 r8 = *reinterpret_cast<const uint4*>(reinterpret_cast<const __nv_bfloat16*>(rp) + j);
                  const uint32_t w[4] = {r8.x, r8.y, r8.z, r8.w};
#pragma unroll
                  for (int q = 0; q < 4; ++q) {
                    const __nv_bfloat162 p = *reinterpret_cast<const __nv_bfloat162*>(&w[q]);
                    f[j + 2 * q] += __low2float(p);
                    f[j + 2 * q + 1] += __high2float(p);
                  }
                }
              }
            }
          }
          if constexpr (sizeof(OutT) == 4) {
#pragma unroll
            for (int q = 0; q < 8; ++q) {
              const int phys = q ^ (row_in_tile & 7);
              *reinterpret_cast<float4*>(cd_row + phys * 16) =
                  make_float4(f[4 * q], f[4 * q + 1], f[4 * q + 2], f[4 * q + 3]);
            }
          } else {
#pragma unroll
            for (int q = 0; q < 4; ++q) {
              const int phys = (s * 4 + q) ^ (row_in_tile & 7);
              *reinterpret_cast<uint4*>(cd_row + phys * 16) =
                  make_uint4(pack_bf16x2(f[8 * q], f[8 * q + 1]), pack_bf16x2(f[8 * q + 2], f[8 * q + 3]),
                             pack_bf16x2(f[8 * q + 4], f[8 * q + 5]), pack_bf16x2(f[8 * q + 6], f[8 * q + 7]));
            }
          }
        }
        if (c + Cfg::EPI_GROUPS >= NUM_CHUNKS) {
          tc_fence_before();
          __syncwarp();
          if (lane == 0) {
            if (kCtaGroup == 2) mbar_arrive_cluster(&tmem_empty_bar[acc], 0);
            else mbar_arrive(&tmem_empty_bar[acc]);
          }
        }
        fence_proxy_async_smem();
        named_bar_sync(bar_id, 128);
        if (ew == 0 && lane == 0) {
          if constexpr (kEpi == EPI_BIAS_ACCUM) {
            int* flag = nullptr;
            if (k_splits > 1) {
              flag = splitk_flags + ((long long)(m_blk * num_n_tiles + n_blk) * kCtaGroup + int(cta_rank)) * Cfg::EPI_GROUPS + wg;
              if (c == wg && chunk > 0) {
                while (ld_acquire_gpu(flag) != chunk) __nanosleep(64);
                fence_proxy_async_all();
              }
            }
            tma_reduce_add_2d(&tm_c, smem_cd_wg + cd_stage * Cfg::CD_STAGE_BYTES, n0 + c * CHUNK_COLS, m0);
            tma_store_commit();
            if (k_splits > 1 && c + Cfg::EPI_GROUPS >= NUM_CHUNKS) {
              tma_store_wait_all<0>();
              fence_proxy_async_all();
              __threadfence();
              st_release_gpu(flag, chunk == k_splits - 1 ? 0 : chunk + 1);
            }
          } else {
            tma_store_2d(&tm_c, smem_cd_wg + cd_stage * Cfg::CD_STAGE_BYTES, n0 + c * CHUNK_COLS, m0);
            tma_store_commit();
          }
        }
        cd_stage ^= 1;
      }
    }
    if (ew == 0 && lane == 0) tma_store_wait_all<0>();
  }

  tc_fence_before();
  if (kCtaGroup == 2) cluster_sync_all(); else __syncthreads();
  if (warp_idx == 2) tmem_dealloc<kCtaGroup>(tmem_base, Cfg::TMEM_COLS);
}

typedef CUresult (*PFN_tmapEncodeTiled)(CUtensorMap*, CUtensorMapDataType, cuuint32_t, void*, const cuuint64_t*,
                                        const cuuint64_t*, const cuuint32_t*, const cuuint32_t*,
                                        CUtensorMapInterleave, CUtensorMapSwizzle, CUtensorMapL2promotion,
                                        CUtensorMapFloatOOBfill);

static PFN_tmapEncodeTiled get_encode_fn() {
  static PFN_tmapEncodeTiled fn = nullptr;
  if (!fn) {
    void* p = nullptr;
    cudaDriverEntryPointQueryResult q;
    if (cudaGetDriverEntryPoint("cuTensorMapEncodeTiled", &p, cudaEnableDefault, &q) != cudaSuccess ||
        q != cudaDriverEntryPointSuccess || !p) {
      set_last_error("cuTensorMapEncodeTiled driver entry point not available");
      return nullptr;
    }
    fn = reinterpret_cast<PFN_tmapEncodeTiled>(p);
  }
  return fn;
}

int make_tmap_2d(CUtensorMap* out, const void* ptr, int elem_bytes, long long rows, long long cols, long long ld,
                 int box_rows, int box_cols) {
  PFN_tmapEncodeTiled enc = get_encode_fn();
  if (!enc) return -3;
  CUtensorMapDataType dt = (elem_bytes == 2) ? CU_TENSOR_MAP_DATA_TYPE_BFLOAT16 : CU_TENSOR_MAP_DATA_TYPE_FLOAT32;
  cuuint64_t dims[2] = {(cuuint64_t)cols, (cuuint64_t)rows};
  cuuint64_t strides[1] = {(cuuint64_t)ld * (cuuint64_t)elem_bytes};
  cuuint32_t box[2] = {(cuuint32_t)box_cols, (cuuint32_t)box_rows};
  cuuint32_t estr[2] = {1, 1};
  if (box_cols * elem_bytes != 128) {
    set_last_error("make_tmap_2d: inner box must span 128 bytes");
    return -1;
  }
  CUresult r = enc(out, dt, 2, const_cast<void*>(ptr), dims, strides, box, estr, CU_TENSOR_MAP_INTERLEAVE_NONE,
                   CU_TENSOR_MAP_SWIZZLE_128B, CU_TENSOR_MAP_L2_PROMOTION_L2_256B,
                   CU_TENSOR_MAP_FLOAT_OOB_FILL_NONE);
  if (r != CUDA_SUCCESS) {
    set_last_error("cuTensorMapEncodeTiled failed with CUresult %d (rows=%lld cols=%lld ld=%lld elem=%d)", (int)r,
                   rows, cols, ld, elem_bytes);
    return -3;
  }
  return 0;
}

template <int kCtaGroup, int kEpi, typename OutT, int kEpiGroups = 2>
static int launch_inst(const CUtensorMap& ta, const CUtensorMap& tb, const CUtensorMap& tc, const float* bias,
                       const void* residual, long long ldr, int M, int N, int K, int num_sms, cudaStream_t stream,
                       float* cand_val = nullptr, int* cand_idx = nullptr, float* lse_part = nullptr,
                       int n_chunks = 1, const LnFold& lf = LnFold(), const ColFilter& cf = ColFilter(), int k_splits = 1,
                       int* splitk_flags = nullptr) {
  using Cfg = GemmCfg<kCtaGroup, kEpiGroups>;
  auto kern = gemm_bf16_tcgen05_kernel<kCtaGroup, kEpi, OutT, kEpiGroups>;
  static bool attr_set[64] = {};
  if (first_use_on_device(attr_set)) {
    SB_CUDA_CHECK(cudaFuncSetAttribute(kern, cudaFuncAttributeMaxDynamicSharedMemorySize, Cfg::SMEM_BYTES));
  }
  const int tile_m = Cfg::BLOCK_M * kCtaGroup;
  const long long num_m_tiles = (M + tile_m - 1) / tile_m;
  const long long num_tiles = num_m_tiles * ((N + Cfg::BLOCK_N - 1) / Cfg::BLOCK_N);
  long long clusters = num_sms / kCtaGroup;
  if (clusters > num_tiles * k_splits) clusters = num_tiles * k_splits;
  if (kEpi == EPI_TOPK && clusters > num_m_tiles * n_chunks) clusters = num_m_tiles * n_chunks;
  if (clusters < 1) clusters = 1;
  cudaLaunchConfig_t cfg = {};
  cfg.gridDim = dim3((unsigned)(clusters * kCtaGroup), 1, 1);
  cfg.blockDim = dim3(Cfg::THREADS, 1, 1);
  cfg.dynamicSmemBytes = Cfg::SMEM_BYTES;
  cfg.stream = stream;
  cudaLaunchAttribute attr[1];
  attr[0].id = cudaLaunchAttributeClusterDimension;
  attr[0].val.clusterDim.x = kCtaGroup;
  attr[0].val.clusterDim.y = 1;
  attr[0].val.clusterDim.z = 1;
  cfg.attrs = attr;
  cfg.numAttrs = 1;
  SB_CUDA_CHECK(cudaLaunchKernelEx(&cfg, kern, ta, tb, tc, bias, reinterpret_cast<const OutT*>(residual), ldr, M, N, K,
                                   cand_val, cand_idx, lse_part, n_chunks, lf, cf, k_splits, splitk_flags));
  return 0;
}

int gemm_topk_chunks(int M, int N, int cta_group, int num_sms) {
  const int cg = (cta_group == 1) ? 1 : 2;
  const int clusters = (num_sms > 0 ? num_sms : 148) / cg;
  const int num_m_tiles = (M + 128 * cg - 1) / (128 * cg);
  const int num_n_tiles = (N + 255) / 256;
  int want = clusters / num_m_tiles;
  if (want < 1) want = 1;
  if (want > num_n_tiles) want = num_n_tiles;
  const int tpc = (num_n_tiles + want - 1) / want;
  return (num_n_tiles + tpc - 1) / tpc;
}

int gemm_bf16_topk(const __nv_bfloat16* A, long long lda, const __nv_bfloat16* W, long long ldw, int M, int N, int K,
                   float* cand_val, int* cand_idx, float* lse_part, int n_chunks, int cta_group, int num_sms,
                   cudaStream_t stream, const ColFilter& cf) {
  if (M <= 0 || N <= 0) return 0;
  if (cf.thr != nullptr && (!cf.thr8 || !cf.cnt || !cf.buf || cf.cap <= 0)) {
    set_last_error("gemm_bf16_topk: column filter needs cnt, buf and a positive capacity");
    return -1;
  }
  if (K % 64 != 0 || K <= 0) {
    set_last_error("gemm_bf16_topk: K must be a positive multiple of 64 (got %d)", K);
    return -1;
  }
  const int num_n_tiles = (N + 255) / 256;
  if (n_chunks < 1 || n_chunks > num_n_tiles ||
      ((num_n_tiles + n_chunks - 1) / n_chunks) * (n_chunks - 1) >= num_n_tiles) {
    set_last_error("gemm_bf16_topk: invalid n_chunks=%d for %d n-tiles", n_chunks, num_n_tiles);
    return -1;
  }
  const int cg = (cta_group == 1) ? 1 : 2;
  CUtensorMap ta, tb;
  int rc;
  if ((rc = make_tmap_2d(&ta, A, 2, M, K, lda, 128, 64))) return rc;
  if ((rc = make_tmap_2d(&tb, W, 2, N, K, ldw, 256 / cg, 64))) return rc;
  const int sms = num_sms > 0 ? num_sms : 148;
  if (cg == 2)
    return launch_inst<2, EPI_TOPK, float>(ta, tb, ta , nullptr, nullptr, 0, M, N, K, sms, stream, cand_val,
                                           cand_idx, lse_part, n_chunks, LnFold(), cf);
  return launch_inst<1, EPI_TOPK, float>(ta, tb, ta , nullptr, nullptr, 0, M, N, K, sms, stream, cand_val,
                                         cand_idx, lse_part, n_chunks, LnFold(), cf);
}

int gemm_bf16(const GemmArgs& g, cudaStream_t stream) {
  if (g.M <= 0) return 0;
  if (g.allow_skinny && gemm_skinny_eligible(g) && !g.lf.stats_in && g.epi != EPI_BIAS_RESIDUAL_STATS)
    return gemm_skinny(g, stream);
  if (g.N % 256 != 0 || g.K % 64 != 0 || g.K <= 0 || g.N <= 0) {
    set_last_error("gemm_bf16: need N %% 256 == 0 and K %% 64 == 0 (got M=%d N=%d K=%d)", g.M, g.N, g.K);
    return -1;
  }
  if (g.epi == EPI_BIAS_RESIDUAL && !g.residual) {
    set_last_error("gemm_bf16: residual epilogue without residual pointer");
    return -1;
  }
  if (!g.bias) {
    set_last_error("gemm_bf16: bias pointer is required");
    return -1;
  }
  const int cg = (g.cta_group == 1) ? 1 : 2;
  const int out_bytes = g.out_fp32 ? 4 : 2;
  CUtensorMap ta, tb, tc;
  int rc;
  if ((rc = make_tmap_2d(&ta, g.A, 2, g.M, g.K, g.lda, 128, 64))) return rc;
  if ((rc = make_tmap_2d(&tb, g.W, 2, g.N, g.K, g.ldw, 256 / cg, 64))) return rc;
  if ((rc = make_tmap_2d(&tc, g.C, out_bytes, g.M, g.N, g.ldc, 128, 128 / out_bytes))) return rc;
  const int sms = g.num_sms > 0 ? g.num_sms : 148;
  int epi = g.epi;
  if (epi == EPI_BIAS_RESIDUAL && g.out_fp32 && g.residual == g.C && g.ldr == g.ldc) epi = EPI_BIAS_ACCUM;
  if (epi == EPI_BIAS_ACCUM && !g.out_fp32) {
    set_last_error("gemm_bf16: accumulate epilogue needs fp32 output");
    return -1;
  }

  if (g.lf.stats_in != nullptr) {
    if ((epi != EPI_BIAS && epi != EPI_BIAS_RELU) || !g.lf.colsum || g.lf.chunks < 1 || g.lf.chunks > 8 ||
        g.K != kLnPartCols * g.lf.chunks) {
      set_last_error("gemm_bf16: folded LayerNorm input needs a bias / bias+ReLU epilogue and K = 128 * chunks <= 1024 "
                     "(K=%d chunks=%d)", g.K, g.lf.chunks);
      return -1;
    }
  }
  if (epi == EPI_BIAS_RESIDUAL_STATS) {
    if (!g.out_fp32 || !g.residual || !g.lf.h_out || !g.lf.stats_out || g.lf.ldh < g.N) {
      set_last_error("gemm_bf16: the residual+statistics epilogue needs fp32 C, a residual, h_out and stats_out");
      return -1;
    }
  } else if (g.lf.h_out != nullptr || g.lf.stats_out != nullptr) {
    set_last_error("gemm_bf16: h_out / stats_out are outputs of EPI_BIAS_RESIDUAL_STATS only");
    return -1;
  }

  if (g.epi_groups == 1) {
    if (cg != 2 || (epi != EPI_BIAS && epi != EPI_BIAS_RELU && epi != EPI_BIAS_ACCUM) || g.lf.stats_in != nullptr) {
      set_last_error("gemm_bf16: epi_groups = 1 is only built for the paired-CTA bias / bias+ReLU / accumulate epilogues");
      return -1;
    }
    if (epi == EPI_BIAS_ACCUM)
      return launch_inst<2, EPI_BIAS_ACCUM, float, 1>(ta, tb, tc, g.bias, g.residual, g.ldr, g.M, g.N, g.K, sms, stream);
    if (g.out_fp32) { set_last_error("gemm_bf16: epi_groups = 1 needs bf16 output for bias / bias+ReLU"); return -1; }
    if (epi == EPI_BIAS)
      return launch_inst<2, EPI_BIAS, __nv_bfloat16, 1>(ta, tb, tc, g.bias, g.residual, g.ldr, g.M, g.N, g.K, sms, stream);
    return launch_inst<2, EPI_BIAS_RELU, __nv_bfloat16, 1>(ta, tb, tc, g.bias, g.residual, g.ldr, g.M, g.N, g.K, sms, stream);
  }

  if (epi == EPI_BIAS_ACCUM && cg == 2 && g.splitk_flags != nullptr) {
    const long long tiles = (long long)((g.M + 255) / 256) * (g.N / 256);
    const long long clusters = sms / 2;
    const int num_kb = g.K / 64;
    int best = 1;
    double best_cost = 1e30;
    for (int ks = 1; ks <= 4; ++ks) {
      if (num_kb / ks < 8) break;
      const double cost = double((tiles * ks + clusters - 1) / clusters) * (double(num_kb) / ks + 8.0);
      if (cost < best_cost * 0.95) { best_cost = cost; best = ks; }
    }
    if (best > 1 && tiles * 2 * 2 <= g.splitk_flags_len)
      return launch_inst<2, EPI_BIAS_ACCUM, float>(ta, tb, tc, g.bias, g.residual, g.ldr, g.M, g.N, g.K, sms, stream, nullptr,
                                                   nullptr, nullptr, 1, LnFold(), ColFilter(), best, g.splitk_flags);
  }

#define SB_DISPATCH(CG, EPI, T)                                                                                   \
  return launch_inst<CG, EPI, T>(ta, tb, tc, g.bias, g.residual, g.ldr, g.M, g.N, g.K, sms, stream, nullptr, nullptr, \
                                 nullptr, 1, g.lf)
#define SB_DISPATCH_EPI(CG, T)                                              \
  switch (epi) {                                                            \
    case EPI_BIAS: SB_DISPATCH(CG, EPI_BIAS, T);                            \
    case EPI_BIAS_RELU: SB_DISPATCH(CG, EPI_BIAS_RELU, T);                  \
    case EPI_BIAS_SILU: SB_DISPATCH(CG, EPI_BIAS_SILU, T);                  \
    case EPI_BIAS_RESIDUAL: SB_DISPATCH(CG, EPI_BIAS_RESIDUAL, T);          \
    case EPI_BIAS_ACCUM: SB_DISPATCH(CG, EPI_BIAS_ACCUM, float);            \
    case EPI_BIAS_RESIDUAL_STATS: SB_DISPATCH(CG, EPI_BIAS_RESIDUAL_STATS, float); \
    default: set_last_error("gemm_bf16: bad epilogue %d", epi); return -1;  \
  }
  if (cg == 2) {
    if (g.out_fp32) { SB_DISPATCH_EPI(2, float) } else { SB_DISPATCH_EPI(2, __nv_bfloat16) }
  } else {
    if (g.out_fp32) { SB_DISPATCH_EPI(1, float) } else { SB_DISPATCH_EPI(1, __nv_bfloat16) }
  }
#undef SB_DISPATCH
#undef SB_DISPATCH_EPI
  return -1;
}

}
```

sonar_b200/csrc/sonar_b200_internal.h:

```cpp
#pragma once

#include <cuda.h>
#include <cuda_bf16.h>
#include <cuda_runtime.h>
#include <stdint.h>

namespace sb {

enum EpiMode { EPI_BIAS = 0, EPI_BIAS_RELU = 1, EPI_BIAS_RESIDUAL = 2, EPI_BIAS_ACCUM = 3, EPI_TOPK = 4, EPI_BIAS_SILU = 5,
               EPI_BIAS_RESIDUAL_STATS = 6 };
constexpr int kTopkCandidates = 16;
enum PoolMode { POOL_MAX = 1, POOL_MEAN = 2, POOL_LAST = 3 };

void set_last_error(const char* fmt, ...);

inline bool first_use_on_device(bool (&flags)[64]) {
  int dev = 0;
  if (cudaGetDevice(&dev) != cudaSuccess || dev < 0 || dev >= 64) return true;
  if (flags[dev]) return false;
  flags[dev] = true;
  return true;
}

constexpr int kLnPartCols = 128;
struct LnFold {
  const float* stats_in = nullptr;
  const float* colsum = nullptr;
  int chunks = 0;
  float eps = 0.f;
  __nv_bfloat16* h_out = nullptr;
  long long ldh = 0;
  float* stats_out = nullptr;
};

struct GemmArgs {
  const __nv_bfloat16* A;
  long long lda;
  const __nv_bfloat16* W;
  long long ldw;
  void* C;
  long long ldc;
  int out_fp32;
  const float* bias;
  const void* residual;
  long long ldr;
  int M, N, K;
  int epi;
  int cta_group;
  int num_sms;
  LnFold lf;
  int allow_skinny = 0;
  int epi_groups = 2;
  int* splitk_flags = nullptr;
  long long splitk_flags_len = 0;
};

int gemm_bf16(const GemmArgs& g, cudaStream_t stream);

bool gemm_skinny_eligible(const GemmArgs& g);
int gemm_skinny(const GemmArgs& g, cudaStream_t stream);

struct ColFilter {
  float* thr = nullptr;
  const float* thr8 = nullptr;
  int* cnt = nullptr;
  uint2* buf = nullptr;
  int cap = 0;
};

int gemm_topk_chunks(int M, int N, int cta_group, int num_sms);
constexpr int kTopkListsPerChunk = 2;
inline int gemm_topk_lists(int n_chunks) { return kTopkListsPerChunk * n_chunks; }
int gemm_bf16_topk(const __nv_bfloat16* A, long long lda, const __nv_bfloat16* W, long long ldw, int M, int N, int K,
                   float* cand_val, int* cand_idx, float* lse_part, int n_chunks, int cta_group, int num_sms,
                   cudaStream_t stream, const ColFilter& cf = ColFilter());

int make_tmap_2d(CUtensorMap* out, const void* ptr, int elem_bytes, long long rows, long long cols, long long ld,
                 int box_rows, int box_cols);

int embed_tokens(const int64_t* ids, long long ids_stride, const int32_t* cu_seqlens, int B, int S,
                 const __nv_bfloat16* embed, long long vocab, const float* pos_table, int pos_rows, int D, float scale,
                 float* x, int* err_flag, cudaStream_t stream, int pos_offset = 0, __nv_bfloat16* h_out = nullptr,
                 float* stats_out = nullptr);

int fold_layernorm_weights(const __nv_bfloat16* W, const float* bias, const float* gamma, const float* beta, int N, int K,
                           __nv_bfloat16* Wf, float* colsum, float* bias_f, cudaStream_t stream);

int layernorm_bf16(const float* x, const float* gamma, const float* beta, float eps, __nv_bfloat16* y, long long T,
                   int D, cudaStream_t stream);

int layernorm_dual(const float* x, const float* gamma, const float* beta, float eps, float* y32, __nv_bfloat16* y16,
                   long long T, int D, cudaStream_t stream);

int attention_packed(const __nv_bfloat16* qkv, const int32_t* cu_seqlens, int B, int max_len, int H,
                     long long total_tokens, int impl, int num_sms, __nv_bfloat16* out, cudaStream_t stream);
int attention_packed_tc(const __nv_bfloat16* qkv, const int32_t* cu_seqlens, int B, int H, long long total_tokens,
                        __nv_bfloat16* out, int num_sms, cudaStream_t stream);

int attention_relpos_tc(const __nv_bfloat16* qkv, const __nv_bfloat16* p, const float* u_bias, const float* v_bias,
                        const int32_t* cu_seqlens, int B, int H, long long total_tokens, int Npad, int S_center,
                        __nv_bfloat16* qu, __nv_bfloat16* qv, __nv_bfloat16* out, int num_sms, cudaStream_t stream);

int ln_pool(const float* x, const int32_t* cu_seqlens, int B, int D, const float* gamma, const float* beta,
            float eps, int apply_ln, int pool_mode, float* out, float* encoded_padded, int S_padded,
            cudaStream_t stream);

}
```

sonar_b200/ops.py:

```python

from __future__ import annotations

from typing import Optional

import torch
from torch import Tensor

from . import _lib

POOLING_MODES = {"max": _lib.SB_POOL_MAX, "mean": _lib.SB_POOL_MEAN, "last": _lib.SB_POOL_LAST}


def _need_cuda(*tensors: Optional[Tensor]) -> None:
    for t in tensors:
        if t is not None and not t.is_cuda:
            raise RuntimeError("sonar_b200 ops run on CUDA tensors only (no CPU fallback exists)")


def _stream() -> int:
    return torch.cuda.current_stream().cuda_stream


def _ptr(t: Optional[Tensor]) -> Optional[int]:
    return None if t is None else t.data_ptr()


def gemm_bf16(a: Tensor, w: Tensor, bias: Tensor, *, epilogue: str = "bias", residual: Optional[Tensor] = None,
              out_dtype: torch.dtype = torch.bfloat16, out: Optional[Tensor] = None, cta_group: int = 2) -> Tensor:
    _need_cuda(a, w, bias, residual, out)
    assert a.dtype == torch.bfloat16 and w.dtype == torch.bfloat16 and bias.dtype == torch.float32
    assert a.dim() == 2 and w.dim() == 2 and a.stride(1) == 1 and w.stride(1) == 1
    m, k = a.shape
    n = w.shape[0]
    assert w.shape[1] == k and bias.numel() == n
    epi = {"bias": _lib.SB_EPI_BIAS, "relu": _lib.SB_EPI_BIAS_RELU, "residual": _lib.SB_EPI_BIAS_RESIDUAL, "silu": 5}[epilogue]
    if out is None:
        out = torch.empty((m, n), dtype=out_dtype, device=a.device)
    assert out.dtype in (torch.bfloat16, torch.float32) and out.stride(1) == 1
    if epilogue == "residual":
        assert residual is not None and residual.dtype == out.dtype and residual.stride(1) == 1
    rc = _lib.load().sb_gemm_bf16(
        a.data_ptr(), a.stride(0), w.data_ptr(), w.stride(0), out.data_ptr(), out.stride(0),
        1 if out.dtype == torch.float32 else 0, bias.data_ptr(), _ptr(residual),
        residual.stride(0) if residual is not None else 0, m, n, k, epi, cta_group, _stream())
    _lib.check(rc, "sb_gemm_bf16")
    return out


def layernorm(x: Tensor, gamma: Tensor, beta: Tensor, eps: float = 1e-5) -> Tensor:
    _need_cuda(x, gamma, beta)
    assert x.dtype == torch.float32 and x.is_contiguous() and x.dim() == 2
    y = torch.empty(x.shape, dtype=torch.bfloat16, device=x.device)
    rc = _lib.load().sb_layernorm(x.data_ptr(), gamma.data_ptr(), beta.data_ptr(), eps, y.data_ptr(),
                                  x.shape[0], x.shape[1], _stream())
    _lib.check(rc, "sb_layernorm")
    return y


def cu_seqlens_of(seq_lens) -> Tensor:
    lens = torch.as_tensor(seq_lens, dtype=torch.int64).cpu()
    cu = torch.zeros(lens.numel() + 1, dtype=torch.int32)
    cu[1:] = torch.cumsum(lens, 0).to(torch.int32)
    return cu


ATTENTION_IMPLS = {"auto": 0, "mma_sync": 1, "tcgen05": 2}


def fold_layernorm(w: Tensor, bias: Tensor, gamma: Tensor, beta: Tensor):
    _need_cuda(w, bias, gamma, beta)
    assert w.dtype == torch.bfloat16 and w.is_contiguous()
    n, k = w.shape
    wf = torch.empty_like(w)
    colsum = torch.empty((n,), dtype=torch.float32, device=w.device)
    bias_f = torch.empty((n,), dtype=torch.float32, device=w.device)
    rc = _lib.load().sb_fold_layernorm(w.data_ptr(), bias.data_ptr(), gamma.data_ptr(), beta.data_ptr(), n, k, wf.data_ptr(),
                                       colsum.data_ptr(), bias_f.data_ptr(), _stream())
    _lib.check(rc, "sb_fold_layernorm")
    return wf, colsum, bias_f


def gemm_residual_stats(a: Tensor, w: Tensor, bias: Tensor, x: Tensor):
    _need_cuda(a, w, bias, x)
    m, k = a.shape
    n = w.shape[0]
    assert x.shape == (m, n) and x.dtype == torch.float32 and x.is_contiguous() and n % 256 == 0
    h = torch.empty((m, n), dtype=torch.bfloat16, device=a.device)
    stats = torch.empty((m, n // 128, 2), dtype=torch.float32, device=a.device)
    rc = _lib.load().sb_gemm_residual_stats(a.data_ptr(), a.stride(0), w.data_ptr(), w.stride(0), x.data_ptr(), n,
                                            bias.data_ptr(), h.data_ptr(), n, stats.data_ptr(), m, n, k, _stream())
    _lib.check(rc, "sb_gemm_residual_stats")
    return h, stats


def gemm_residual_splitk(a: Tensor, w: Tensor, bias: Tensor, x: Tensor, counters: Tensor) -> Tensor:
    _need_cuda(a, w, bias, x, counters)
    m, k = a.shape
    n = w.shape[0]
    assert x.shape == (m, n) and x.dtype == torch.float32 and x.is_contiguous() and counters.dtype == torch.int32
    rc = _lib.load().sb_gemm_residual_splitk(a.data_ptr(), a.stride(0), w.data_ptr(), w.stride(0), x.data_ptr(), n,
                                             bias.data_ptr(), m, n, k, counters.data_ptr(), counters.numel(), _stream())
    _lib.check(rc, "sb_gemm_residual_splitk")
    return x


def gemm_ln_consumer(a: Tensor, wf: Tensor, bias_f: Tensor, colsum: Tensor, stats: Tensor, eps: float = 1e-5,
                     relu: bool = False) -> Tensor:
    _need_cuda(a, wf, bias_f, colsum, stats)
    m, k = a.shape
    n = wf.shape[0]
    out = torch.empty((m, n), dtype=torch.bfloat16, device=a.device)
    rc = _lib.load().sb_gemm_ln_consumer(a.data_ptr(), a.stride(0), wf.data_ptr(), wf.stride(0), out.data_ptr(), n,
                                         bias_f.data_ptr(), colsum.data_ptr(), stats.data_ptr(), eps, m, n, k,
                                         1 if relu else 0, _stream())
    _lib.check(rc, "sb_gemm_ln_consumer")
    return out


def attention(qkv: Tensor, cu_seqlens: Tensor, max_len: int, num_heads: int, impl: str = "auto") -> Tensor:
    _need_cuda(qkv, cu_seqlens)
    assert qkv.dtype == torch.bfloat16 and qkv.is_contiguous() and cu_seqlens.dtype == torch.int32
    t = qkv.shape[0]
    d = 64 * num_heads
    assert qkv.shape[1] == 3 * d
    out = torch.empty((t, d), dtype=torch.bfloat16, device=qkv.device)
    rc = _lib.load().sb_attention(qkv.data_ptr(), cu_seqlens.data_ptr(), cu_seqlens.numel() - 1, max_len,
                                  num_heads, t, ATTENTION_IMPLS[impl], out.data_ptr(), _stream())
    _lib.check(rc, "sb_attention")
    return out


def embed(ids: Tensor, cu_seqlens: Tensor, table: Tensor, pos_table: Tensor, scale: float, total_tokens: int) -> Tensor:
    _need_cuda(ids, cu_seqlens, table, pos_table)
    assert ids.dtype == torch.int64 and ids.stride(1) == 1 and table.dtype == torch.bfloat16
    b, s = ids.shape
    d = table.shape[1]
    x = torch.empty((total_tokens, d), dtype=torch.float32, device=ids.device)
    err = torch.zeros(1, dtype=torch.int32, device=ids.device)
    rc = _lib.load().sb_embed(ids.data_ptr(), ids.stride(0), cu_seqlens.data_ptr(), b, s, table.data_ptr(),
                              table.shape[0], pos_table.data_ptr(), pos_table.shape[0], d, scale, x.data_ptr(),
                              err.data_ptr(), _stream())
    _lib.check(rc, "sb_embed")
    if int(err.item()) != 0:
        raise ValueError("sb_embed: token id outside [0, vocab_size)")
    return x


def pool_packed(x: Tensor, cu_seqlens: Tensor, pooling: str, *, gamma: Optional[Tensor] = None,
                beta: Optional[Tensor] = None, eps: float = 1e-5, encoded_seq_len: int = 0):
    _need_cuda(x, cu_seqlens, gamma, beta)
    assert x.dtype == torch.float32 and x.is_contiguous()
    b = cu_seqlens.numel() - 1
    d = x.shape[1]
    out = torch.empty((b, d), dtype=torch.float32, device=x.device)
    enc = torch.empty((b, encoded_seq_len, d), dtype=torch.float32, device=x.device) if encoded_seq_len > 0 else None
    rc = _lib.load().sb_pool(x.data_ptr(), cu_seqlens.data_ptr(), b, d, _ptr(gamma), _ptr(beta), eps,
                             1 if gamma is not None else 0, POOLING_MODES[pooling.lower()], out.data_ptr(),
                             _ptr(enc), encoded_seq_len, _stream())
    _lib.check(rc, "sb_pool")
    return (out, enc) if enc is not None else out
```

sonar_b200/text_encoder.py:

```python

from __future__ import annotations

import ctypes as C
import math
from dataclasses import dataclass, field
from enum import Enum
from pathlib import Path
from typing import Dict, List, Optional, Union

import numpy as np
import torch
from torch import Tensor

from . import _lib, ops
from .sequence import PaddingMask, SequenceBatch, SonarEncoderOutput


class Pooling(Enum):

    MAX = 1
    MEAN = 2
    LAST = 3
    ATTENTION = 4


@dataclass
class VocabularyInfo:
    size: int
    unk_idx: Optional[int] = None
    bos_idx: Optional[int] = None
    eos_idx: Optional[int] = None
    pad_idx: Optional[int] = None


@dataclass
class SonarTextEncoderConfig:

    model_dim: int = 1024
    max_seq_len: int = 512
    vocab_info: VocabularyInfo = field(
        default_factory=lambda: VocabularyInfo(size=256206, unk_idx=1, bos_idx=2, eos_idx=3, pad_idx=1))
    num_encoder_layers: int = 24
    num_decoder_layers: int = 24
    num_encoder_attn_heads: int = 16
    num_decoder_attn_heads: int = 16
    ffn_inner_dim: int = 1024 * 8
    pooling: str = "mean"
    embedding_dim: Optional[int] = None
    decoder_ffn_inner_dim: Optional[int] = None
    activation_fn: str = "ReLU"
    layernorm_embedding: bool = False
    no_scale_embedding: bool = False
    no_token_positional_embeddings: bool = False
    learned_pos: bool = False
    emb_dropout_p: float = 0.1
    attention_dropout_p: float = 0.1
    activation_dropout_p: float = 0.1
    normalize_before: bool = False
    _from_fairseq: bool = True


def sonar_text_encoder_config(arch: str = "basic", **overrides) -> SonarTextEncoderConfig:
    if arch == "basic":
        cfg = SonarTextEncoderConfig()
    elif arch == "small":
        cfg = SonarTextEncoderConfig(
            vocab_info=VocabularyInfo(size=32005, unk_idx=1, bos_idx=2, eos_idx=3, pad_idx=1),
            num_encoder_layers=6, num_decoder_layers=6, ffn_inner_dim=1024 * 4)
    else:
        raise ValueError(f"unknown sonar text encoder arch {arch!r}")
    for k, v in overrides.items():
        if not hasattr(cfg, k):
            raise TypeError(f"unknown config field {k!r}")
        setattr(cfg, k, v)
    return cfg


def sinusoidal_position_table(num_pos: int, dim: int, legacy_pad_idx: int) -> Tensor:
    half = dim // 2
    start = legacy_pad_idx + 1
    steps = torch.arange(start, start + num_pos, dtype=torch.float32)
    freq = torch.exp(torch.arange(half, dtype=torch.float32) * -(math.log(10000.0) / (half - 1)))
    ang = steps[:, None] * freq[None, :]
    return torch.cat([torch.sin(ang), torch.cos(ang)], dim=1).contiguous()


class _PosEncoderInfo:
    def __init__(self, max_seq_len: int) -> None:
        self.max_seq_len = max_seq_len


class _FrontendInfo:

    def __init__(self, max_seq_len: int, model_dim: int) -> None:
        self.pos_encoder = _PosEncoderInfo(max_seq_len)
        self.model_dim = model_dim


def _check_supported(cfg: SonarTextEncoderConfig) -> None:
    bad = []
    if cfg.pooling.lower() not in ("mean", "max", "last"):
        bad.append(f"pooling={cfg.pooling!r} (attention pooling is not on the B200 hot path yet)")
    if cfg.activation_fn != "ReLU":
        bad.append(f"activation_fn={cfg.activation_fn!r}")
    if cfg.layernorm_embedding or cfg.no_token_positional_embeddings or cfg.learned_pos:
        bad.append("layernorm_embedding / no_token_positional_embeddings / learned_pos")
    if cfg.embedding_dim not in (None, cfg.model_dim):
        bad.append("embedding_dim != model_dim")
    if cfg.model_dim != 64 * cfg.num_encoder_attn_heads:
        bad.append("head_dim != 64")
    if bad:
        raise NotImplementedError("sonar_b200 text encoder does not support: " + "; ".join(bad))


class B200TextEncoderModel(torch.nn.Module):

    def __init__(self, config: SonarTextEncoderConfig, state_dict: Dict[str, Tensor],
                 device: Union[str, torch.device] = "cuda", *, cta_group: int = 2, ln_fold: Union[bool, int] = False,
                 epi_groups: Optional[int] = None) -> None:
        super().__init__()
        if epi_groups is None:
            epi_groups = 2 if int(ln_fold) else 1
        self.ln_fold = int(ln_fold)
        self.epi_groups = int(epi_groups)
        _check_supported(config)
        self.config = config
        self.model_dim = config.model_dim
        self.pooling = getattr(Pooling, config.pooling.upper())
        dev = torch.device(device)
        if dev.type != "cuda":
            raise RuntimeError("B200TextEncoderModel needs a CUDA device (there is no CPU path)")
        if dev.index is None:
            dev = torch.device("cuda", torch.cuda.current_device())
        self.device = dev
        pad_idx = config.vocab_info.pad_idx if config.vocab_info.pad_idx is not None else 1
        max_len = config.max_seq_len + (pad_idx + 1 if config._from_fairseq else 0)
        self.encoder_frontend = _FrontendInfo(max_len, config.model_dim)
        self._lib = _lib.load()

        sd = state_dict
        d, L = config.model_dim, config.num_encoder_layers

        def bf(t: Tensor) -> Tensor:
            return t.detach().to(device=dev, dtype=torch.bfloat16).contiguous()

        def f32(t: Tensor) -> Tensor:
            return t.detach().to(device=dev, dtype=torch.float32).contiguous()

        embed = sd["encoder_frontend.embed.weight"]
        if embed.shape != (config.vocab_info.size, d):
            raise ValueError(f"embedding shape {tuple(embed.shape)} != ({config.vocab_info.size}, {d})")
        self.register_buffer("embed", bf(embed), persistent=False)
        self.register_buffer("pos_table", sinusoidal_position_table(max_len, d, pad_idx).to(dev), persistent=False)
        self.register_buffer("final_ln_g", f32(sd["layer_norm.weight"]), persistent=False)
        self.register_buffer("final_ln_b", f32(sd["layer_norm.bias"]), persistent=False)
        self._layer_bufs: List[Dict[str, Tensor]] = []
        for i in range(L):
            p = f"encoder.layers.{i}."
            a = p + "self_attn."
            bufs = {
                "wqkv": bf(torch.cat([sd[a + "q_proj.weight"], sd[a + "k_proj.weight"], sd[a + "v_proj.weight"]], 0)),
                "bqkv": f32(torch.cat([sd[a + "q_proj.bias"], sd[a + "k_proj.bias"], sd[a + "v_proj.bias"]], 0)),
                "wo": bf(sd[a + "output_proj.weight"]), "bo": f32(sd[a + "output_proj.bias"]),
                "w1": bf(sd[p + "ffn.inner_proj.weight"]), "b1": f32(sd[p + "ffn.inner_proj.bias"]),
                "w2": bf(sd[p + "ffn.output_proj.weight"]), "b2": f32(sd[p + "ffn.output_proj.bias"]),
                "ln1_g": f32(sd[p + "self_attn_layer_norm.weight"]), "ln1_b": f32(sd[p + "self_attn_layer_norm.bias"]),
                "ln2_g": f32(sd[p + "ffn_layer_norm.weight"]), "ln2_b": f32(sd[p + "ffn_layer_norm.bias"]),
            }
            for k, v in bufs.items():
                self.register_buffer(f"l{i}_{k}", v, persistent=False)
            self._layer_bufs.append(bufs)

        cfg_c = _lib.SbEncoderConfig(
            model_dim=d, num_layers=L, num_heads=config.num_encoder_attn_heads, ffn_inner_dim=config.ffn_inner_dim,
            vocab_size=config.vocab_info.size, pos_rows=max_len, pooling=self.pooling.value, ln_eps=1e-5,
            embed_scale=1.0 if config.no_scale_embedding else math.sqrt(d), cta_group=cta_group, num_sms=0,
            ln_fold=int(ln_fold), epi_groups=int(epi_groups))
        layers_c = (_lib.SbLayerWeights * max(L, 1))()
        for i, bufs in enumerate(self._layer_bufs):
            for k, v in bufs.items():
                setattr(layers_c[i], k, v.data_ptr())
        w_c = _lib.SbEncoderWeights(embed=self.embed.data_ptr(), pos_table=self.pos_table.data_ptr(),
                                    final_ln_g=self.final_ln_g.data_ptr(), final_ln_b=self.final_ln_b.data_ptr(),
                                    layers=layers_c)
        handle = C.c_void_p()
        with torch.cuda.device(dev):
            _lib.check(self._lib.sb_encoder_create(C.byref(cfg_c), C.byref(w_c), C.byref(handle)), "sb_encoder_create")
        self._handle = handle
        self._workspace: Optional[Tensor] = None
        self.return_encoded_seqs = False

    @classmethod
    def from_checkpoint(cls, path: Union[str, Path], config: Optional[SonarTextEncoderConfig] = None,
                        device: Union[str, torch.device] = "cuda", **kw) -> "B200TextEncoderModel":
        ckpt = torch.load(str(path), map_location="cpu", weights_only=True)
        sd = ckpt["model"] if "model" in ckpt else ckpt
        return cls(config or sonar_text_encoder_config("basic"), sd, device, **kw)

    @property
    def dtype(self) -> torch.dtype:
        return torch.bfloat16

    def __del__(self) -> None:
        try:
            if getattr(self, "_handle", None):
                self._lib.sb_encoder_destroy(self._handle)
                self._handle = None
        except Exception:
            pass

    def _ensure_workspace(self, batch: int, tokens: int) -> Tensor:
        need = C.c_size_t()
        _lib.check(self._lib.sb_encoder_workspace_bytes(self._handle, batch, tokens, C.byref(need)),
                   "sb_encoder_workspace_bytes")
        if self._workspace is None or self._workspace.numel() < need.value:
            self._workspace = None
            self._workspace = torch.empty(int(need.value * 1.1) + 4096, dtype=torch.uint8, device=self.device)
        return self._workspace

    @torch.inference_mode()
    def forward(self, batch: SequenceBatch) -> SonarEncoderOutput:
        seqs = batch.seqs
        if seqs.dim() != 2:
            raise ValueError("expected token ids of shape [N, S]")
        if not seqs.is_cuda:
            seqs = seqs.to(self.device, non_blocking=True)
        if seqs.dtype != torch.int64:
            seqs = seqs.to(torch.int64)
        if seqs.stride(1) != 1:
            seqs = seqs.contiguous()
        n, s = seqs.shape
        pm = batch.padding_mask
        if pm is not None:
            lens_np = np.ascontiguousarray(pm.seq_lens_host, dtype=np.int32)
            lens_c = lens_np.ctypes.data_as(C.POINTER(C.c_int32))
            tokens = int(lens_np.sum(dtype=np.int64))
        else:
            lens_c = None
            tokens = n * s
        ws = self._ensure_workspace(n, max(tokens, 1))
        out = torch.empty((n, self.model_dim), dtype=torch.float32, device=self.device)
        enc = (torch.empty((n, s, self.model_dim), dtype=torch.float32, device=self.device)
               if self.return_encoded_seqs else None)
        with torch.cuda.device(self.device):
            rc = self._lib.sb_encoder_forward(
                self._handle, seqs.data_ptr(), seqs.stride(0), lens_c, n, s, out.data_ptr(),
                enc.data_ptr() if enc is not None else None, ws.data_ptr(), ws.numel(),
                torch.cuda.current_stream(self.device).cuda_stream)
        _lib.check(rc, "sb_encoder_forward")
        return SonarEncoderOutput(encoded_seqs=enc, sentence_embeddings=out, padding_mask=pm)

    def profile_ffn1(self, start: Optional[torch.cuda.Event], stop: Optional[torch.cuda.Event]) -> None:
        _lib.check(self._lib.sb_encoder_profile_ffn1(self._handle, start.cuda_event if start is not None else None,
                                                     stop.cuda_event if stop is not None else None),
                   "sb_encoder_profile_ffn1")

    def check_inputs(self) -> None:
        if self._workspace is None:
            return
        rc = self._lib.sb_encoder_check_inputs(self._handle, self._workspace.data_ptr(),
                                               torch.cuda.current_stream(self.device).cuda_stream)
        _lib.check(rc, "sb_encoder_check_inputs")

    @staticmethod
    def static_pooling(seqs: Tensor, padding_mask: Optional[PaddingMask], pooling: Pooling) -> Tensor:
        if pooling == Pooling.ATTENTION:
            raise NotImplementedError(pooling)
        if not seqs.is_cuda:
            raise RuntimeError("static_pooling runs on CUDA tensors only")
        n, s, d = seqs.shape
        lens = padding_mask.seq_lens_host if padding_mask is not None else [s] * n
        valid = (torch.arange(s)[None, :] < torch.tensor(lens)[:, None]).to(seqs.device)
        packed = seqs.float()[valid].contiguous()
        cu = ops.cu_seqlens_of(lens).to(seqs.device)
        return ops.pool_packed(packed, cu, pooling.name).to(seqs.dtype)
```

Baseline: 8750.

## Share A-operand tiles across two CTA pairs via TMA multicast in 4-CTA clusters

Adds a kPairs=2 GEMM variant that requests 4-CTA preferred clusters. Two paired-CTA groups working on the same M tile but different N tiles each load half of the A tile and multicast it to both pairs, halving A global/L2 traffic. The stage-empty barriers now expect two arrivals, and commits and TMEM-empty arrivals target the right pair leader. It is on by default for paired-CTA bias/ReLU/accumulate GEMMs without LN fold, but it couples the two pairs' pipelines and relies on the preferred cluster shape being granted.

```diff
diff --git a/include/sonar_b200.h b/include/sonar_b200.h
--- a/include/sonar_b200.h
+++ b/include/sonar_b200.h
@@ -39,7 +39,10 @@
   int32_t num_sms;
   int32_t ln_fold;
   int32_t epi_groups;
+  int32_t cluster_pairs;
 } SbEncoderConfig;
+
+#define SB_ENCODER_DEFAULT_CLUSTER_PAIRS 2
 
 typedef struct SbLayerWeights {
   const void* wqkv;
@@ -98,7 +101,9 @@
 
 int sb_gemm_bf16(const void* A, int64_t lda, const void* W, int64_t ldw, void* C, int64_t ldc, int32_t out_fp32,
                  const float* bias, const void* residual, int64_t ldr, int32_t M, int32_t N, int32_t K, int32_t epi,
-                 int32_t cta_group, void* stream);
+                 int32_t cta_group, int32_t cluster_pairs, int32_t num_sms, void* stream);
+
+int sb_gemm_max_active_clusters(int32_t cluster_ctas, int32_t* clusters);
 
 int sb_layernorm(const float* x, const float* gamma, const float* beta, float eps, void* y, int64_t T, int32_t D,
                  void* stream);
diff --git a/sonar_b200/_lib.py b/sonar_b200/_lib.py
--- a/sonar_b200/_lib.py
+++ b/sonar_b200/_lib.py
@@ -19,6 +19,7 @@
         ("ffn_inner_dim", C.c_int32), ("vocab_size", C.c_int64), ("pos_rows", C.c_int32),
         ("pooling", C.c_int32), ("ln_eps", C.c_float), ("embed_scale", C.c_float),
         ("cta_group", C.c_int32), ("num_sms", C.c_int32), ("ln_fold", C.c_int32), ("epi_groups", C.c_int32),
+        ("cluster_pairs", C.c_int32),
     ]
 
 
@@ -95,7 +96,8 @@
     "sb_encoder_check_inputs": (C.c_int, [C.c_void_p, C.c_void_p, C.c_void_p]),
     "sb_gemm_bf16": (C.c_int, [C.c_void_p, C.c_int64, C.c_void_p, C.c_int64, C.c_void_p, C.c_int64,
                                C.c_int32, C.c_void_p, C.c_void_p, C.c_int64, C.c_int32, C.c_int32,
-                               C.c_int32, C.c_int32, C.c_int32, C.c_void_p]),
+                               C.c_int32, C.c_int32, C.c_int32, C.c_int32, C.c_int32, C.c_void_p]),
+    "sb_gemm_max_active_clusters": (C.c_int, [C.c_int32, C.POINTER(C.c_int32)]),
     "sb_layernorm": (C.c_int, [C.c_void_p, C.c_void_p, C.c_void_p, C.c_float, C.c_void_p, C.c_int64,
                                C.c_int32, C.c_void_p]),
     "sb_attention": (C.c_int, [C.c_void_p, C.c_void_p, C.c_int32, C.c_int32, C.c_int32, C.c_int64, C.c_int32,
diff --git a/sonar_b200/csrc/common.cuh b/sonar_b200/csrc/common.cuh
--- a/sonar_b200/csrc/common.cuh
+++ b/sonar_b200/csrc/common.cuh
@@ -34,6 +34,12 @@
   uint32_t r;
   asm volatile("mov.u32 %0, %%cluster_ctarank;" : "=r"(r));
   return r;
+}
+
+__device__ __forceinline__ uint32_t cluster_nctarank() {
+  uint32_t n;
+  asm volatile("mov.u32 %0, %%cluster_nctarank;" : "=r"(n));
+  return n;
 }
 
 __device__ __forceinline__ bool elect_one() {
@@ -148,6 +154,16 @@
       "cp.async.bulk.tensor.2d.cta_group::2.shared::cluster.global.mbarrier::complete_tx::bytes [%0], [%1, {%3, "
       "%4}], [%2];" ::"r"(smem_u32(smem_dst)),
       "l"(reinterpret_cast<uint64_t>(m)), "r"(bar_addr), "r"(c0), "r"(c1)
+      : "memory");
+}
+
+__device__ __forceinline__ void tma_load_2d_cta2_multicast(void* smem_dst, const CUtensorMap* m, uint64_t* bar, int c0,
+                                                           int c1, uint16_t cta_mask) {
+  uint32_t bar_addr = smem_u32(bar) & 0xFEFFFFFFu;
+  asm volatile(
+      "cp.async.bulk.tensor.2d.shared::cluster.global.tile.mbarrier::complete_tx::bytes.multicast::cluster.cta_group::2 "
+      "[%0], [%1, {%3, %4}], [%2], %5;" ::"r"(smem_u32(smem_dst)),
+      "l"(reinterpret_cast<uint64_t>(m)), "r"(bar_addr), "r"(c0), "r"(c1), "h"(cta_mask)
       : "memory");
 }
 
diff --git a/sonar_b200/csrc/encoder.cu b/sonar_b200/csrc/encoder.cu
--- a/sonar_b200/csrc/encoder.cu
+++ b/sonar_b200/csrc/encoder.cu
@@ -113,6 +113,10 @@
     set_last_error("sb_encoder_create: epi_groups = 1 (the one-warpgroup epilogue kept for A/B runs) needs ln_fold = 0 and paired CTAs");
     return SB_ERR_INVALID;
   }
+  if (cfg->cluster_pairs < 0 || cfg->cluster_pairs > 2 || (cfg->cluster_pairs == 2 && cfg->cta_group == 1)) {
+    set_last_error("sb_encoder_create: cluster_pairs must be 0, 1 or 2, and 2 needs paired CTAs (got %d)", cfg->cluster_pairs);
+    return SB_ERR_INVALID;
+  }
   if (cfg->num_layers < 0 || cfg->pos_rows <= 0 || cfg->vocab_size <= 0) {
     set_last_error("sb_encoder_create: bad num_layers / pos_rows / vocab_size");
     return SB_ERR_INVALID;
@@ -290,6 +294,7 @@
   g.num_sms = e->num_sms;
   g.M = (int)T;
   g.epi_groups = (e->cfg.epi_groups == 1) ? 1 : 2;
+  g.cluster_pairs = e->cfg.cluster_pairs != 0 ? e->cfg.cluster_pairs : (g.cta_group == 2 ? SB_ENCODER_DEFAULT_CLUSTER_PAIRS : 1);
   LnFold consume;
   consume.stats_in = w.ln_stats;
   consume.chunks = D / kLnPartCols;
@@ -396,8 +401,12 @@
 
 int sb_gemm_bf16(const void* A, int64_t lda, const void* W, int64_t ldw, void* C, int64_t ldc, int32_t out_fp32,
                  const float* bias, const void* residual, int64_t ldr, int32_t M, int32_t N, int32_t K, int32_t epi,
-                 int32_t cta_group, void* stream) {
+                 int32_t cta_group, int32_t cluster_pairs, int32_t num_sms, void* stream) {
   if (!A || !W || !C) { set_last_error("sb_gemm_bf16: null pointer"); return SB_ERR_INVALID; }
+  if (cluster_pairs < 0 || cluster_pairs > 2 || num_sms < 0) {
+    set_last_error("sb_gemm_bf16: cluster_pairs must be 0, 1 or 2 and num_sms >= 0 (got %d, %d)", cluster_pairs, num_sms);
+    return SB_ERR_INVALID;
+  }
   GemmArgs g;
   g.A = reinterpret_cast<const __nv_bfloat16*>(A); g.lda = lda;
   g.W = reinterpret_cast<const __nv_bfloat16*>(W); g.ldw = ldw;
@@ -405,11 +414,16 @@
   g.M = M; g.N = N; g.K = K; g.epi = epi;
   g.cta_group = cta_group == 1 ? 1 : 2;
   g.allow_skinny = (cta_group == 0);
+  g.cluster_pairs = cluster_pairs == 2 ? 2 : 1;
   int dev = 0, sms = 0;
   SB_CUDA_CHECK(cudaGetDevice(&dev));
   SB_CUDA_CHECK(cudaDeviceGetAttribute(&sms, cudaDevAttrMultiProcessorCount, dev));
-  g.num_sms = sms;
+  g.num_sms = num_sms > 0 ? num_sms : sms;
   return gemm_bf16(g, reinterpret_cast<cudaStream_t>(stream));
+}
+
+int sb_gemm_max_active_clusters(int32_t cluster_ctas, int32_t* clusters) {
+  return gemm_max_active_clusters(cluster_ctas, clusters);
 }
 
 int sb_fold_layernorm(const void* W, const float* bias, const float* gamma, const float* beta, int32_t N, int32_t K,
diff --git a/sonar_b200/csrc/gemm_tcgen05.cu b/sonar_b200/csrc/gemm_tcgen05.cu
--- a/sonar_b200/csrc/gemm_tcgen05.cu
+++ b/sonar_b200/csrc/gemm_tcgen05.cu
@@ -3,6 +3,8 @@
 #include "sonar_b200_internal.h"
 
 #include <math_constants.h>
+
+#include <algorithm>
 
 namespace sb {
 
@@ -80,7 +82,7 @@
   }
 }
 
-template <int kCtaGroup, int kEpi, typename OutT, int kEpiGroups>
+template <int kCtaGroup, int kEpi, typename OutT, int kEpiGroups, int kPairs>
 __global__ void __launch_bounds__(GemmCfg<kCtaGroup, kEpiGroups>::THREADS, 1)
 gemm_bf16_tcgen05_kernel(const __grid_constant__ CUtensorMap tm_a, const __grid_constant__ CUtensorMap tm_b,
                          const __grid_constant__ CUtensorMap tm_c, const float* __restrict__ bias,
@@ -88,6 +90,7 @@
                          int* __restrict__ cand_idx, float* __restrict__ lse_part, int n_chunks, const LnFold lf,
                          const ColFilter cf, int k_splits, int* __restrict__ splitk_flags) {
   constexpr bool kSweep = (kEpi == EPI_TOPK);
+  static_assert(kPairs == 1 || (kPairs == 2 && kCtaGroup == 2 && !kSweep), "A-sharing is built for paired CTAs only");
   using Cfg = GemmCfg<kCtaGroup, kEpiGroups>;
   extern __shared__ uint8_t smem_raw[];
   uint8_t* smem = reinterpret_cast<uint8_t*>((reinterpret_cast<uintptr_t>(smem_raw) + 1023) & ~uintptr_t(1023));
@@ -102,7 +105,12 @@
 
   const int warp_idx = threadIdx.x >> 5;
   const int lane = threadIdx.x & 31;
-  const uint32_t cta_rank = (kCtaGroup == 2) ? cluster_ctarank() : 0u;
+  const uint32_t cluster_rank = (kCtaGroup == 2) ? cluster_ctarank() : 0u;
+  const uint32_t cta_rank = (kPairs == 2) ? (cluster_rank & 1u) : cluster_rank;
+  const uint32_t pair_in_cluster = (kPairs == 2) ? (cluster_rank >> 1) : 0u;
+  const bool share_a = (kPairs == 2) && cluster_nctarank() == 4;
+  const uint16_t pair_mask = (kPairs == 2) ? uint16_t(0x3u << (2 * pair_in_cluster)) : uint16_t(0x3u);
+  const uint32_t leader_rank = (kPairs == 2) ? (cluster_rank & ~1u) : 0u;
   const bool is_leader = (cta_rank == 0);
 
   if (kCtaGroup == 2) cluster_sync_all();
@@ -115,7 +123,7 @@
   if (warp_idx == 1 && lane == 0) {
     for (int i = 0; i < Cfg::STAGES; ++i) {
       mbar_init(&full_bar[i], 1);
-      mbar_init(&empty_bar[i], 1);
+      mbar_init(&empty_bar[i], share_a ? 2 : 1);
     }
     for (int i = 0; i < 2; ++i) {
       mbar_init(&tmem_full_bar[i], 1);
@@ -154,7 +162,20 @@
           mbar_wait(&empty_bar[stage], phase ^ 1);
           if (is_leader) mbar_arrive_expect_tx(&full_bar[stage], (Cfg::A_BYTES + Cfg::B_BYTES) * kCtaGroup);
           if (kCtaGroup == 2) {
-            tma_load_2d_cta2(smem_a + stage * Cfg::A_BYTES, &tm_a, &full_bar[stage], kb * Cfg::BLOCK_K, m0);
+            if constexpr (kPairs == 2) {
+              uint8_t* a_dst = smem_a + stage * Cfg::A_BYTES;
+              constexpr int HALF = Cfg::BLOCK_M / 2;
+              if (share_a) {
+                tma_load_2d_cta2_multicast(a_dst + pair_in_cluster * (Cfg::A_BYTES / 2), &tm_a, &full_bar[stage],
+                                           kb * Cfg::BLOCK_K, m0 + int(pair_in_cluster) * HALF,
+                                           uint16_t((1u << cta_rank) | (1u << (cta_rank + 2))));
+              } else {
+                tma_load_2d_cta2(a_dst, &tm_a, &full_bar[stage], kb * Cfg::BLOCK_K, m0);
+                tma_load_2d_cta2(a_dst + Cfg::A_BYTES / 2, &tm_a, &full_bar[stage], kb * Cfg::BLOCK_K, m0 + HALF);
+              }
+            } else {
+              tma_load_2d_cta2(smem_a + stage * Cfg::A_BYTES, &tm_a, &full_bar[stage], kb * Cfg::BLOCK_K, m0);
+            }
             tma_load_2d_cta2(smem_b + stage * Cfg::B_BYTES, &tm_b, &full_bar[stage], kb * Cfg::BLOCK_K, n0);
           } else {
             tma_load_2d(smem_a + stage * Cfg::A_BYTES, &tm_a, &full_bar[stage], kb * Cfg::BLOCK_K, m0);
@@ -191,8 +212,8 @@
               const uint64_t b_desc = (uint64_t(desc_hi) << 32) | uint64_t(b_lo + 2 * k);
               umma_bf16<kCtaGroup>(d_tmem, a_desc, b_desc, idesc, ((kb - kb0) | k) != 0 ? 1u : 0u);
             }
-            umma_commit<kCtaGroup>(&empty_bar[stage]);
-            if (kb == kb1 - 1) umma_commit<kCtaGroup>(&tmem_full_bar[acc]);
+            umma_commit<kCtaGroup>(&empty_bar[stage], share_a ? uint16_t(0xF) : pair_mask);
+            if (kb == kb1 - 1) umma_commit<kCtaGroup>(&tmem_full_bar[acc], pair_mask);
           }
           __syncwarp();
           if (++stage == Cfg::STAGES) { stage = 0; phase ^= 1; }
@@ -364,7 +385,7 @@
         tc_fence_before();
         __syncwarp();
         if (lane == 0) {
-          if (kCtaGroup == 2) mbar_arrive_cluster(&tmem_empty_bar[acc], 0);
+          if (kCtaGroup == 2) mbar_arrive_cluster(&tmem_empty_bar[acc], leader_rank);
           else mbar_arrive(&tmem_empty_bar[acc]);
         }
         if (last_in_item && grow < M) {
@@ -505,7 +526,7 @@
           tc_fence_before();
           __syncwarp();
           if (lane == 0) {
-            if (kCtaGroup == 2) mbar_arrive_cluster(&tmem_empty_bar[acc], 0);
+            if (kCtaGroup == 2) mbar_arrive_cluster(&tmem_empty_bar[acc], leader_rank);
             else mbar_arrive(&tmem_empty_bar[acc]);
           }
         }
@@ -589,14 +610,14 @@
   return 0;
 }
 
-template <int kCtaGroup, int kEpi, typename OutT, int kEpiGroups = 2>
+template <int kCtaGroup, int kEpi, typename OutT, int kEpiGroups = 2, int kPairs = 1>
 static int launch_inst(const CUtensorMap& ta, const CUtensorMap& tb, const CUtensorMap& tc, const float* bias,
                        const void* residual, long long ldr, int M, int N, int K, int num_sms, cudaStream_t stream,
                        float* cand_val = nullptr, int* cand_idx = nullptr, float* lse_part = nullptr,
                        int n_chunks = 1, const LnFold& lf = LnFold(), const ColFilter& cf = ColFilter(), int k_splits = 1,
                        int* splitk_flags = nullptr) {
   using Cfg = GemmCfg<kCtaGroup, kEpiGroups>;
-  auto kern = gemm_bf16_tcgen05_kernel<kCtaGroup, kEpi, OutT, kEpiGroups>;
+  auto kern = gemm_bf16_tcgen05_kernel<kCtaGroup, kEpi, OutT, kEpiGroups, kPairs>;
   static bool attr_set[64] = {};
   if (first_use_on_device(attr_set)) {
     SB_CUDA_CHECK(cudaFuncSetAttribute(kern, cudaFuncAttributeMaxDynamicSharedMemorySize, Cfg::SMEM_BYTES));
@@ -608,20 +629,51 @@
   if (clusters > num_tiles * k_splits) clusters = num_tiles * k_splits;
   if (kEpi == EPI_TOPK && clusters > num_m_tiles * n_chunks) clusters = num_m_tiles * n_chunks;
   if (clusters < 1) clusters = 1;
+  if (kPairs == 2 && (clusters % 2 != 0 || ((N + Cfg::BLOCK_N - 1) / Cfg::BLOCK_N) % 2 != 0 || k_splits != 1)) {
+    set_last_error("gemm_bf16: A-sharing needs an even number of CTA pairs and of n-tiles (pairs=%lld N=%d)", clusters, N);
+    return -1;
+  }
   cudaLaunchConfig_t cfg = {};
   cfg.gridDim = dim3((unsigned)(clusters * kCtaGroup), 1, 1);
   cfg.blockDim = dim3(Cfg::THREADS, 1, 1);
   cfg.dynamicSmemBytes = Cfg::SMEM_BYTES;
   cfg.stream = stream;
-  cudaLaunchAttribute attr[1];
+  cudaLaunchAttribute attr[2];
   attr[0].id = cudaLaunchAttributeClusterDimension;
   attr[0].val.clusterDim.x = kCtaGroup;
   attr[0].val.clusterDim.y = 1;
   attr[0].val.clusterDim.z = 1;
+  attr[1].id = cudaLaunchAttributePreferredClusterDimension;
+  attr[1].val.preferredClusterDim.x = 2 * kCtaGroup;
+  attr[1].val.preferredClusterDim.y = 1;
+  attr[1].val.preferredClusterDim.z = 1;
+  cfg.attrs = attr;
+  cfg.numAttrs = kPairs == 2 ? 2 : 1;
+  SB_CUDA_CHECK(cudaLaunchKernelEx(&cfg, kern, ta, tb, tc, bias, reinterpret_cast<const OutT*>(residual), ldr, M, N, K,
+                                   cand_val, cand_idx, lse_part, n_chunks, lf, cf, k_splits, splitk_flags));
+  return 0;
+}
+
+int gemm_max_active_clusters(int cluster_ctas, int* clusters) {
+  if ((cluster_ctas != 2 && cluster_ctas != 4) || !clusters) {
+    set_last_error("gemm_max_active_clusters: cluster_ctas must be 2 or 4");
+    return -1;
+  }
+  using Cfg = GemmCfg<2, 1>;
+  auto kern = gemm_bf16_tcgen05_kernel<2, EPI_BIAS_RELU, __nv_bfloat16, 1, 2>;
+  SB_CUDA_CHECK(cudaFuncSetAttribute(kern, cudaFuncAttributeMaxDynamicSharedMemorySize, Cfg::SMEM_BYTES));
+  cudaLaunchConfig_t cfg = {};
+  cfg.gridDim = dim3(unsigned(cluster_ctas * 64), 1, 1);
+  cfg.blockDim = dim3(Cfg::THREADS, 1, 1);
+  cfg.dynamicSmemBytes = Cfg::SMEM_BYTES;
+  cudaLaunchAttribute attr[1];
+  attr[0].id = cudaLaunchAttributeClusterDimension;
+  attr[0].val.clusterDim.x = unsigned(cluster_ctas);
+  attr[0].val.clusterDim.y = 1;
+  attr[0].val.clusterDim.z = 1;
   cfg.attrs = attr;
   cfg.numAttrs = 1;
-  SB_CUDA_CHECK(cudaLaunchKernelEx(&cfg, kern, ta, tb, tc, bias, reinterpret_cast<const OutT*>(residual), ldr, M, N, K,
-                                   cand_val, cand_idx, lse_part, n_chunks, lf, cf, k_splits, splitk_flags));
+  SB_CUDA_CHECK(cudaOccupancyMaxActiveClusters(clusters, kern, &cfg));
   return 0;
 }
 
@@ -717,18 +769,32 @@
     return -1;
   }
 
+  long long pairs = std::min<long long>(sms / 2, (long long)((g.M + 255) / 256) * (g.N / 256));
+  if (pairs < 1) pairs = 1;
+  const bool share_a = g.cluster_pairs == 2 && cg == 2 && !g.lf.stats_in && g.splitk_flags == nullptr &&
+                       (((epi == EPI_BIAS || epi == EPI_BIAS_RELU) && !g.out_fp32) || epi == EPI_BIAS_ACCUM) &&
+                       (g.N / 256) % 2 == 0 && pairs % 2 == 0;
+  if (share_a && (rc = make_tmap_2d(&ta, g.A, 2, g.M, g.K, g.lda, 64, 64))) return rc;
+#define SB_LAUNCH_PAIRED(EPI, T, EG)                                                                                  \
+  return share_a ? launch_inst<2, EPI, T, EG, 2>(ta, tb, tc, g.bias, g.residual, g.ldr, g.M, g.N, g.K, sms, stream) \
+                 : launch_inst<2, EPI, T, EG, 1>(ta, tb, tc, g.bias, g.residual, g.ldr, g.M, g.N, g.K, sms, stream)
+
   if (g.epi_groups == 1) {
     if (cg != 2 || (epi != EPI_BIAS && epi != EPI_BIAS_RELU && epi != EPI_BIAS_ACCUM) || g.lf.stats_in != nullptr) {
       set_last_error("gemm_bf16: epi_groups = 1 is only built for the paired-CTA bias / bias+ReLU / accumulate epilogues");
       return -1;
     }
-    if (epi == EPI_BIAS_ACCUM)
-      return launch_inst<2, EPI_BIAS_ACCUM, float, 1>(ta, tb, tc, g.bias, g.residual, g.ldr, g.M, g.N, g.K, sms, stream);
+    if (epi == EPI_BIAS_ACCUM) SB_LAUNCH_PAIRED(EPI_BIAS_ACCUM, float, 1);
     if (g.out_fp32) { set_last_error("gemm_bf16: epi_groups = 1 needs bf16 output for bias / bias+ReLU"); return -1; }
-    if (epi == EPI_BIAS)
-      return launch_inst<2, EPI_BIAS, __nv_bfloat16, 1>(ta, tb, tc, g.bias, g.residual, g.ldr, g.M, g.N, g.K, sms, stream);
-    return launch_inst<2, EPI_BIAS_RELU, __nv_bfloat16, 1>(ta, tb, tc, g.bias, g.residual, g.ldr, g.M, g.N, g.K, sms, stream);
-  }
+    if (epi == EPI_BIAS) SB_LAUNCH_PAIRED(EPI_BIAS, __nv_bfloat16, 1);
+    SB_LAUNCH_PAIRED(EPI_BIAS_RELU, __nv_bfloat16, 1);
+  }
+  if (share_a) {
+    if (epi == EPI_BIAS_ACCUM) SB_LAUNCH_PAIRED(EPI_BIAS_ACCUM, float, 2);
+    if (epi == EPI_BIAS) SB_LAUNCH_PAIRED(EPI_BIAS, __nv_bfloat16, 2);
+    SB_LAUNCH_PAIRED(EPI_BIAS_RELU, __nv_bfloat16, 2);
+  }
+#undef SB_LAUNCH_PAIRED
 
   if (epi == EPI_BIAS_ACCUM && cg == 2 && g.splitk_flags != nullptr) {
     const long long tiles = (long long)((g.M + 255) / 256) * (g.N / 256);
diff --git a/sonar_b200/csrc/sonar_b200_internal.h b/sonar_b200/csrc/sonar_b200_internal.h
--- a/sonar_b200/csrc/sonar_b200_internal.h
+++ b/sonar_b200/csrc/sonar_b200_internal.h
@@ -53,9 +53,11 @@
   int epi_groups = 2;
   int* splitk_flags = nullptr;
   long long splitk_flags_len = 0;
+  int cluster_pairs = 1;
 };
 
 int gemm_bf16(const GemmArgs& g, cudaStream_t stream);
+int gemm_max_active_clusters(int cluster_ctas, int* clusters);
 
 bool gemm_skinny_eligible(const GemmArgs& g);
 int gemm_skinny(const GemmArgs& g, cudaStream_t stream);
diff --git a/sonar_b200/ops.py b/sonar_b200/ops.py
--- a/sonar_b200/ops.py
+++ b/sonar_b200/ops.py
@@ -1,6 +1,7 @@
 
 from __future__ import annotations
 
+import ctypes
 from typing import Optional
 
 import torch
@@ -26,7 +27,8 @@
 
 
 def gemm_bf16(a: Tensor, w: Tensor, bias: Tensor, *, epilogue: str = "bias", residual: Optional[Tensor] = None,
-              out_dtype: torch.dtype = torch.bfloat16, out: Optional[Tensor] = None, cta_group: int = 2) -> Tensor:
+              out_dtype: torch.dtype = torch.bfloat16, out: Optional[Tensor] = None, cta_group: int = 2,
+              cluster_pairs: int = 1, num_sms: int = 0) -> Tensor:
     _need_cuda(a, w, bias, residual, out)
     assert a.dtype == torch.bfloat16 and w.dtype == torch.bfloat16 and bias.dtype == torch.float32
     assert a.dim() == 2 and w.dim() == 2 and a.stride(1) == 1 and w.stride(1) == 1
@@ -42,9 +44,15 @@
     rc = _lib.load().sb_gemm_bf16(
         a.data_ptr(), a.stride(0), w.data_ptr(), w.stride(0), out.data_ptr(), out.stride(0),
         1 if out.dtype == torch.float32 else 0, bias.data_ptr(), _ptr(residual),
-        residual.stride(0) if residual is not None else 0, m, n, k, epi, cta_group, _stream())
+        residual.stride(0) if residual is not None else 0, m, n, k, epi, cta_group, cluster_pairs, num_sms, _stream())
     _lib.check(rc, "sb_gemm_bf16")
     return out
+
+
+def gemm_max_active_clusters(cluster_ctas: int) -> int:
+    n = ctypes.c_int32(0)
+    _lib.check(_lib.load().sb_gemm_max_active_clusters(cluster_ctas, ctypes.byref(n)), "sb_gemm_max_active_clusters")
+    return int(n.value)
 
 
 def layernorm(x: Tensor, gamma: Tensor, beta: Tensor, eps: float = 1e-5) -> Tensor:
diff --git a/sonar_b200/text_encoder.py b/sonar_b200/text_encoder.py
--- a/sonar_b200/text_encoder.py
+++ b/sonar_b200/text_encoder.py
@@ -117,7 +117,7 @@
 
     def __init__(self, config: SonarTextEncoderConfig, state_dict: Dict[str, Tensor],
                  device: Union[str, torch.device] = "cuda", *, cta_group: int = 2, ln_fold: Union[bool, int] = False,
-                 epi_groups: Optional[int] = None) -> None:
+                 epi_groups: Optional[int] = None, cluster_pairs: int = 0) -> None:
         super().__init__()
         if epi_groups is None:
             epi_groups = 2 if int(ln_fold) else 1
@@ -175,7 +175,7 @@
             model_dim=d, num_layers=L, num_heads=config.num_encoder_attn_heads, ffn_inner_dim=config.ffn_inner_dim,
             vocab_size=config.vocab_info.size, pos_rows=max_len, pooling=self.pooling.value, ln_eps=1e-5,
             embed_scale=1.0 if config.no_scale_embedding else math.sqrt(d), cta_group=cta_group, num_sms=0,
-            ln_fold=int(ln_fold), epi_groups=int(epi_groups))
+            ln_fold=int(ln_fold), epi_groups=int(epi_groups), cluster_pairs=int(cluster_pairs))
         layers_c = (_lib.SbLayerWeights * max(L, 1))()
         for i, bufs in enumerate(self._layer_bufs):
             for k, v in bufs.items():
```

Measured after the change: 8965, median of 6. 2.5% higher.
